# robin-karlsson0/pc-accumulation-lib

Hardware: AMD Instinct MI355X
Metric: Mpoints/s projected+accumulated and BEV frames/s @256x256; 1/2/4/8 GPU (higher is better)
Workload: dtype f64; 1 GPU; KITTI-360 single forward cam, 120k pts/frame, 200 m horizon (~201 live frames, 5169634 stored pts), one 256x256x21 BEV per integrated frame; points_per_frame=120000, bev_px=256, view_m=80

## Files before the change

### include/pca.h

```cpp
#ifndef PCA_H
#define PCA_H

#include <stdint.h>

#ifdef __cplusplus
extern "C" {
#endif

#define PCA_VERSION 2

typedef struct pca_ctx pca_ctx;

typedef struct {
    double *x, *y, *z;
    float *intensity;
    uint32_t *rgbs;
    int32_t *inst;
    uint8_t *dyn;
    int64_t capacity;
    uint32_t *frame_box;
} pca_store;

#define PCA_STATUS_STORE_OVERFLOW 1u
#define PCA_STATUS_UV_OUT_OF_IMAGE 2u
#define PCA_STATUS_NEGATIVE_INTENSITY 4u
#define PCA_STATUS_LOOKBACK_TIMEOUT 8u
#define PCA_STATUS_LANES_BISECT_CAP 16u

int pca_version(void);
int pca_ctx_create(int device, pca_ctx **out);
void pca_ctx_destroy(pca_ctx *ctx);
const char *pca_last_error(pca_ctx *ctx);
int pca_status(pca_ctx *ctx, void *stream, uint32_t *status_out);
int pca_status_peek(pca_ctx *ctx, uint32_t *status_out);
const uint32_t *pca_status_mirror(pca_ctx *ctx);

typedef struct {
    const float *pts;
    const uint8_t *rgb;
    const uint8_t *sem;
    const uint8_t *sem_gt;
    int32_t n;
    int32_t reserved;
} pca_kitti_frame;

int pca_kitti_project_sample_filter(pca_ctx *ctx, const pca_kitti_frame *frames, int n_frames, const double P[12],
                                    int H, int W, const uint64_t filter_mask[4], const pca_store *store,
                                    int64_t *frame_off , int first_slot, void *stream);

#define PCA_SAMPLE_NEAREST 0
#define PCA_SAMPLE_BILINEAR 1
int pca_kitti_project_sample_filter_ex(pca_ctx *ctx, const pca_kitti_frame *frames, int n_frames, const double P[12],
                                       int H, int W, const uint64_t filter_mask[4], const pca_store *store,
                                       int64_t *frame_off , int first_slot, int sample_mode, void *stream);

int pca_nusc_sample_filter_transform(pca_ctx *ctx, const double *pc, const int64_t *cam_idx, int32_t n,
                                     const uint8_t *imgs, const uint8_t *sems, int ncam, int H, int W,
                                     const double T[16], const uint64_t filter_mask[4], const pca_store *store,
                                     int64_t *frame_off , int slot, void *stream);
int pca_nusc_sample_filter_transform_ex(pca_ctx *ctx, const double *pc, const int64_t *cam_idx, int32_t n,
                                        const uint8_t *imgs, const uint8_t *sems, int ncam, int H, int W,
                                        const double T[16], const uint64_t filter_mask[4], const pca_store *store,
                                        int64_t *frame_off , int slot, int sample_mode, void *stream);

typedef struct {
    const double *pc;
    const int64_t *cam_idx;
    const uint8_t *imgs;
    const uint8_t *sems;
    int32_t n;
    int32_t reserved;
    const double *T;
} pca_nusc_frame;
int pca_nusc_sample_filter_transform_batch(pca_ctx *ctx, const pca_nusc_frame *frames, int n_frames, int ncam, int H, int W,
                                           const uint64_t filter_mask[4], const pca_store *store, int64_t *frame_off ,
                                           int first_slot, int sample_mode, void *stream);

int pca_sample_bilinear(pca_ctx *ctx, const double *map , int H, int W, const double *uv , int32_t n,
                        double *out , void *stream);

int pca_nusc_project_cams(pca_ctx *ctx, const double *pc_lidar, int32_t n, const double T_ego_from_lidar[16],
                          const double T_glob_from_ego[16], const double *T_cam_from_glob, const double *K,
                          const double *wh, int ncam, double *pc_in_ego, double *uv, int64_t *cam_idx,
                          void *stream);

#define PCA_NUSC_MAX_SWEEPS 32
#define PCA_NUSC_MAX_SWEEP_BOXES 4096
#define PCA_NUSC_MAX_SWEEP_TILES 16384
typedef struct {
    int32_t row0, n_rows;
    int32_t box0, n_boxes;
    float lag, sweep;
    double T[12];
} pca_nusc_sweep;
typedef struct {
    double inv[12];
    double size[3];
    int32_t cls;
    int32_t track_key;
} pca_nusc_sweep_box;
int64_t pca_nusc_merge_sweeps_workspace_bytes(int64_t n_points, int n_boxes);
int pca_nusc_merge_sweeps(pca_ctx *ctx, const float *raw , int64_t n_points, const pca_nusc_sweep *sweeps,
                          int n_sweeps, const pca_nusc_sweep_box *boxes, int n_boxes, float center_radius,
                          double inside_limit, void *workspace , int64_t workspace_bytes,
                          float *points_out , int32_t *tally_out , void *stream);

int pca_retransform(pca_ctx *ctx, const pca_store *store, const int64_t *frame_off , int slot_begin,
                    int slot_end, const double *Ts, int n_T, void *stream);

int pca_retransform_batch_tail(pca_ctx *ctx, const pca_store *store, const int64_t *frame_off , int first_slot,
                               int n_frames, const double *Ts, void *stream);

int pca_mark_dynamic(pca_ctx *ctx, const pca_store *store, const int64_t *frame_off , const int32_t *slots,
                     const int32_t *inst_idx, int n_pairs, void *stream);

int64_t pca_voxel_dedup_workspace_bytes(int64_t max_points, int n_slots);
int pca_voxel_dedup(pca_ctx *ctx, const pca_store *store, int64_t *frame_off , int slot_begin, int slot_end,
                    double voxel_size, int64_t max_points, void *workspace , int64_t workspace_bytes,
                    void *stream);

int64_t pca_icp_workspace_bytes(int32_t max_points);
int pca_icp_register(pca_ctx *ctx, const float *src_pts , int32_t n_src, const float *tgt_pts ,
                     int32_t n_tgt, double max_corr_dist, const double init[16], int max_iter, double rel_fitness,
                     double rel_rmse, void *workspace , int64_t workspace_bytes, double T_out[16],
                     double *fitness, double *rmse, int *iterations, void *stream);

typedef struct {
    double origin[3];
    double R[9];
    double dx, dy;
    double view;
    double height_filter;
    double int_scaler, int_sep_scaler, int_mid_threshold;
    double rgb_fill;
    int32_t px;
    int32_t road_class;
    uint64_t dynobj_mask[4];
    int32_t intensity_div255;
    int32_t pad;
} pca_bev_params;

int64_t pca_bev_workspace_bytes(int64_t max_points, int px);

int pca_bev_generate(pca_ctx *ctx, const pca_store *store, const double *intensity64,
                     const int64_t *frame_off , int slot_begin, int slot_split, int slot_end,
                     int64_t max_points, const pca_bev_params *prm, const double *pending_T, int pending_slot_end,
                     void *workspace , int64_t workspace_bytes, double *planes ,
                     uint16_t *planes_f16 , void *stream);

#define PCA_BEV_EXTRA_PLANES 3
int pca_bev_generate_ex(pca_ctx *ctx, const pca_store *store, const double *intensity64,
                        const int64_t *frame_off , int slot_begin, int slot_split, int slot_end,
                        int64_t max_points, const pca_bev_params *prm, const double *pending_T, int pending_slot_end,
                        void *workspace , int64_t workspace_bytes, double *planes ,
                        uint16_t *planes_f16 , double *extra_planes , void *stream);

#define PCA_BEV_MAX_CHAIN 4
int pca_bev_generate_chain(pca_ctx *ctx, const pca_store *store, const double *intensity64,
                           const int64_t *frame_off , int slot_begin, int slot_split, int slot_end,
                           int64_t max_points, const pca_bev_params *prm, const double *pending_Ts,
                           const int *pending_slot_ends, int n_pending, int write_back, void *workspace ,
                           int64_t workspace_bytes, double *planes , uint16_t *planes_f16 ,
                           double *extra_planes , void *stream);

typedef struct {
    int32_t slot_begin, slot_split, slot_end, reserved;
    pca_bev_params prm;
    double *planes;
    uint16_t *planes_f16;
} pca_bev_job;
int pca_bev_generate_many(pca_ctx *ctx, const pca_store *store, const double *intensity64 ,
                          const int64_t *frame_off , const pca_bev_job *jobs, int n_jobs, int64_t max_points,
                          void *workspace , int64_t workspace_bytes, void *stream);

#define PCA_BEV_MAX_CLASS_GROUPS 16
typedef struct { uint64_t mask[4]; } pca_class_group;
int64_t pca_bev_class_workspace_bytes(int64_t max_points, int px);
int pca_bev_class_planes(pca_ctx *ctx, const pca_store *store, const int64_t *frame_off ,
                         int slot_begin, int slot_split, int slot_end, int64_t max_points,
                         const pca_bev_params *prm,
                         const pca_class_group *groups, int n_groups,
                         const double *pending_Ts, const int *pending_slot_ends, int n_pending,
                         void *workspace , int64_t workspace_bytes,
                         double *prob      ,
                         uint16_t *prob_f16,
                         uint32_t *counts  ,
                         void *stream);

int64_t pca_bev_elev_workspace_bytes(int64_t max_points, int px);
int pca_bev_elev_partition(pca_ctx *ctx, const pca_store *store, const int64_t *frame_off ,
                           int slot_begin, int slot_end, int64_t max_points,
                           const pca_bev_params *prm, double elev_thresh, int include_dyn,
                           const double *pending_Ts, const int *pending_slot_ends, int n_pending,
                           void *workspace , int64_t workspace_bytes,
                           double *elev      ,
                           uint8_t *observed ,
                           uint8_t *flags    ,
                           int64_t *counts   ,
                           void *stream);

int pca_image_to_nchw_f32(pca_ctx *ctx, const uint8_t *rgb , int H, int W, const float mean[3], const float std[3],
                          float *out , void *stream);

int pca_bev_warp(pca_ctx *ctx, const uint16_t *planes_f16 , uint16_t *out_f16 , int n_planes, int px,
                 double a_1, double a_2, double b_1, double b_2, void *stream);

int pca_host_ego_to_grid(const double *full, int F, const double R[9], double dx, double dy, double view, int px,
                         double *rows, int32_t *start);

typedef struct {
    double origin[3];
    double R[9];
    double dx, dy, view;
    int32_t px, reserved;
} pca_lane_view;
int64_t pca_lanes_workspace_bytes(int64_t n_vertices, int n_samples, int64_t cap_rows);
int pca_lanes_transform(pca_ctx *ctx, double *xyz , int64_t P, const double T[16], void *stream);
int pca_lanes_to_grid(pca_ctx *ctx, const double *xyz , const int32_t *vertex_lane , const int32_t *start ,
                      int64_t P, int32_t L, const pca_lane_view *views , int S, int64_t cap_rows,
                      double *rows , int32_t *row_lane , int64_t *n_rows , void *ws,
                      void *stream);

typedef struct pca_host_track pca_host_track;
typedef struct {
    const void *pts;
    const void *rgb;
    const void *sem;
    const void *sem_gt;
    int32_t n;
    uint32_t host_mask;
} pca_kitti_obs;
int pca_kitti_integrate(pca_ctx *ctx, const pca_kitti_obs *obs, const double P[12], int H, int W,
                        const uint64_t filter_mask[4], const pca_store *store, int64_t *frame_off , int slot,
                        int sample_mode, pca_host_track *track, const double *T_new_prev, double horizon, int64_t *evicted,
                        double *path_length, void *stream);
void pca_host_camera_cone(const double P[12], int H, int W, double cone[15]);
int pca_host_view_hull(int F, const double *then , const float *box , const double *cone ,
                       const double now[12], const pca_bev_params *prm, int *first, int *last);
int pca_bev_bin_range(pca_ctx *ctx, int slot_first, int slot_last_plus1);
int pca_bev_view_hint(pca_ctx *ctx, int slot0, int F, const double *then, const float *box, const double *cone, const double now[12],
                      const pca_bev_params *prm);
void pca_f32_box_decode(const uint32_t *rows , int n, float *box );

int pca_debug_bev_level1(const pca_ctx *ctx, int out[4]);
int pca_debug_icp_layout(int32_t n_src, int32_t n_tgt, int64_t out[16]);

int pca_k1_defer(pca_ctx *ctx, int on);
int pca_k1_flush(pca_ctx *ctx);
int pca_kitti_generate_bev(pca_ctx *ctx, const pca_store *store, const int64_t *frame_off , int slot_begin,
                           int slot_split, int slot_end, int64_t max_points, const pca_bev_params *prm,
                           const double *pending_Ts, const int *pending_slot_ends, int n_pending, int write_back,
                           void *workspace , int64_t workspace_bytes, uint16_t *planes_f16 ,
                           void *host_planes , const pca_host_track *track, double *traj_rows,
                           int32_t *traj_start, int32_t *n_rows, void *stream);

typedef struct {
    const pca_kitti_obs *obs; const double *P; int32_t H, W; const uint64_t *filter_mask; const pca_store *store;
    int64_t *frame_off; int32_t slot, sample_mode; pca_host_track *track; const double *T_new_prev; double horizon;
    int64_t evicted; double path_length; void *stream;
} pca_kitti_integrate_args;
int pca_kitti_integrate_v(pca_ctx *ctx, pca_kitti_integrate_args *a);
typedef struct {
    const pca_store *store; const int64_t *frame_off; int32_t slot_begin, slot_split, slot_end, pad0; int64_t max_points;
    const pca_bev_params *prm; const double *pending_Ts; const int *pending_slot_ends; int32_t n_pending, write_back;
    void *workspace; int64_t workspace_bytes; uint16_t *planes_f16; void *host_planes; const pca_host_track *track;
    double *traj_rows; int32_t *traj_start; int32_t n_rows, pad1; void *stream;
    int32_t hint_slot0, hint_F; const double *hint_then; const float *hint_box; const double *hint_cone; const double *hint_now;
    int32_t hinted, pad2;
} pca_kitti_generate_bev_args;
int pca_kitti_generate_bev_v(pca_ctx *ctx, pca_kitti_generate_bev_args *a);

int pca_host_stage_h2d(int n, const void *const *src, void *const *pinned, void *const *dev, const int64_t *bytes,
                       void *stream);

int pca_host_d2h_async(pca_ctx *ctx, const void *dev, void *pinned, int64_t bytes, void *stream);
int pca_host_d2h_wait(pca_ctx *ctx, int ticket);

#define PCA_DEFLATE_CHUNK_MAX 32768
#define PCA_DEFLATE_MAX_CHUNKS (1 << 20)
#define PCA_DEFLATE_BOUND(n) ((9 * (int64_t)(n) + 7) / 8 + 16)
typedef struct { int64_t offset; int32_t length; int32_t reserved; } pca_deflate_chunk;
int64_t pca_deflate_workspace_bytes(int64_t n_chunks);
int pca_deflate_chunks(pca_ctx *ctx, const void *src , const pca_deflate_chunk *chunk_table , int64_t n_chunks,
                       void *out , uint32_t *out_sizes , uint32_t *out_crcs , void *workspace ,
                       void *stream);
uint32_t pca_host_crc32_combine(uint32_t crc_a, uint32_t crc_b, int64_t len_b);
int64_t pca_host_gzip_assemble(int32_t n_pieces, const void *const *piece, const int64_t *piece_bytes, const int64_t *raw_bytes,
                               const uint32_t *crc, void *out, int64_t out_cap);

typedef struct pca_host_track pca_host_track;
int pca_host_gemv4_probe(void *cblas_dgemv64, int mode, const double *T , const double *x , int64_t n,
                         double *y );
int pca_host_gemv4_mode(int mode);
int pca_host_incr_probe(void *cblas_dgemv64, const double *d, int64_t n, int64_t r0, int64_t r1, double *out);
int pca_host_incr_blocks(int on);
int pca_host_track_create(pca_host_track **out, void *cblas_dgemv64);
void pca_host_track_destroy(pca_host_track *t);
int64_t pca_host_track_len(const pca_host_track *t);
int64_t pca_host_track_n_segments(const pca_host_track *t);
const double *pca_host_track_poses(const pca_host_track *t);
const double *pca_host_track_segments(const pca_host_track *t);
int pca_host_track_set(pca_host_track *t, const double *poses , int64_t n, const double *segs, int64_t nd);
int pca_host_track_transform(pca_host_track *t, const double T[16]);
int pca_host_track_append(pca_host_track *t, const double pose[3]);
int pca_host_track_push_segment(pca_host_track *t, double *path_length);
int pca_host_track_incr(pca_host_track *t, double *out);
int64_t pca_host_track_evict_beyond(pca_host_track *t, double horizon, double path_length);
int64_t pca_host_track_step(pca_host_track *t, const double T_new_prev[16], double horizon, double *path_length);
int64_t pca_host_track_trigger(pca_host_track *t, double bev_horizon, int64_t previous_idx, double min_step);

enum {
    PCA_K_KITTI = 0, PCA_K_NUSC, PCA_K_PROJECT_CAMS, PCA_K_RETRANSFORM, PCA_K_MARK_DYNAMIC,
    PCA_K_BEV_BIN, PCA_K_BEV_SCAN, PCA_K_BEV_SCATTER, PCA_K_BEV_CELLS, PCA_K_BEV_CELLS_HEAVY, PCA_K_DEDUP, PCA_K_BEV_UNIT, PCA_K_ICP,
    PCA_K_BEV_CLASS_BIN, PCA_K_BEV_CLASS_CELLS, PCA_K_BEV_ELEV_BIN, PCA_K_BEV_ELEV_CELLS, PCA_K_COUNT
};
int pca_profile_enable(pca_ctx *ctx, int on);
int pca_profile_read(pca_ctx *ctx, int kernel_id, double *total_ms, int64_t *launches);

#ifdef __cplusplus
}
#endif
#endif
```

### pc-accumulation-lib_amd/csrc/pca_session.hip

```cpp
#include <vector>

#include "pca_common.h"

int pca_stage_copy(const void *const *src, void *const *dst, const int64_t *bytes, int n);

extern "C" {

int pca_kitti_integrate(pca_ctx *ctx, const pca_kitti_obs *obs, const double P[12], int H, int W,
                        const uint64_t filter_mask[4], const pca_store *store, int64_t *frame_off, int slot, int sample_mode,
                        pca_host_track *track, const double *T_new_prev, double horizon, int64_t *evicted,
                        double *path_length, void *stream)
{
    if (!ctx) return -1;
    if (!obs || obs->n < 0 || !P || !filter_mask || !store || !frame_off) { ctx->err = "kitti_integrate: bad arguments"; return -1; }
    if (track && (!T_new_prev || !evicted || !path_length)) { ctx->err = "kitti_integrate: the pose track needs T_new_prev and its outputs"; return -1; }
    hipStream_t s = (hipStream_t)stream;
    PCA_CHECK(ctx, hipSetDevice(ctx->device));
    if (pca_k1_flush_pending(ctx)) return -1;
    const void *in[4] = {obs->pts, obs->rgb, obs->sem, obs->sem_gt};
    const int64_t size[4] = {16ll * obs->n, 3ll * H * W, 1ll * H * W, 1ll * obs->n};
    const void *dev[4] = {in[0], in[1], in[2], in[3]};
    int64_t off[4] = {0, 0, 0, 0}, total = 0;
    for (int k = 0; k < 4; ++k) {
        if (!(in[k] && ((obs->host_mask >> k) & 1u))) continue;
        if (size[k] > 0) { off[k] = total; total += pca_align256(size[k]); }
        else dev[k] = nullptr;
    }
    pca_ctx::Stage *slot_st = nullptr;
    if (total > 0) {
        pca_ctx::Stage &st = ctx->stage[ctx->stage_next++ % PCA_STAGE_DEPTH];
        if (st.busy) { PCA_CHECK(ctx, hipEventSynchronize(st.done)); st.busy = false; }
        if (st.cap < total) {
            if (st.pin) PCA_CHECK(ctx, hipHostFree(st.pin));
            if (st.dev) PCA_CHECK(ctx, hipFree(st.dev));
            st.pin = st.dev = nullptr; st.cap = 0;
            const int64_t cap = total + total / 4;
            PCA_CHECK(ctx, hipHostMalloc(&st.pin, (size_t)cap));
            PCA_CHECK(ctx, hipMalloc(&st.dev, (size_t)cap));
            st.cap = cap;
        }
        if (!st.done) PCA_CHECK(ctx, hipEventCreateWithFlags(&st.done, hipEventDisableTiming));
        const void *src[4]; void *dst[4]; int64_t bytes[4]; int m = 0;
        for (int k = 0; k < 4; ++k)
            if (in[k] && ((obs->host_mask >> k) & 1u) && size[k] > 0) {
                src[m] = in[k]; dst[m] = (char *)st.pin + off[k]; bytes[m] = size[k]; ++m;
                dev[k] = (char *)st.dev + off[k];
            }
        pca_stage_copy(src, dst, bytes, m);
        const int64_t side_min = PCA_ENV_ONCE("PCA_H2D_SIDE_MIN", 256ll << 10);
        if (total >= side_min) {
            if (!ctx->h2d_stream[0]) PCA_CHECK(ctx, hipStreamCreateWithFlags(&ctx->h2d_stream[0], hipStreamNonBlocking));
            if (!ctx->h2d_done[0]) PCA_CHECK(ctx, hipEventCreateWithFlags(&ctx->h2d_done[0], hipEventDisableTiming));
            PCA_CHECK(ctx, hipMemcpyAsync(st.dev, st.pin, (size_t)total, hipMemcpyHostToDevice, ctx->h2d_stream[0]));
            PCA_CHECK(ctx, hipEventRecord(ctx->h2d_done[0], ctx->h2d_stream[0]));
            PCA_CHECK(ctx, hipStreamWaitEvent(s, ctx->h2d_done[0], 0));
        } else {
            PCA_CHECK(ctx, hipMemcpyAsync(st.dev, st.pin, (size_t)total, hipMemcpyHostToDevice, s));
        }
        slot_st = &st;
    }
    pca_kitti_frame fr;
    fr.pts = (const float *)dev[0]; fr.rgb = (const uint8_t *)dev[1]; fr.sem = (const uint8_t *)dev[2];
    fr.sem_gt = (const uint8_t *)dev[3]; fr.n = obs->n; fr.reserved = 0;
    const bool plain = obs->n > 0 && sample_mode == PCA_SAMPLE_NEAREST && (fr.sem_gt || ((int64_t)H * W * 3 >= 4 && fr.rgb && fr.sem)) &&
                       obs->n <= (1 << 20);
    if (ctx->k1_defer && plain) {
        pca_ctx::K1Pending &pd = ctx->k1_pend;
        pd.fr = fr;
        for (int i = 0; i < 12; ++i) pd.P[i] = P[i];
        pd.H = H; pd.W = W;
        for (int i = 0; i < 4; ++i) pd.filt[i] = filter_mask[i];
        pd.store = *store; pd.frame_off = frame_off; pd.slot = slot; pd.sample_mode = sample_mode; pd.stream = s;
        pd.stage_idx = slot_st ? (int)(slot_st - ctx->stage) : -1;
        pd.valid = true;
    } else {
        const int rc = pca_kitti_project_sample_filter_ex(ctx, &fr, 1, P, H, W, filter_mask, store, frame_off, slot, sample_mode, stream);
        if (slot_st) {
            const hipError_t e = hipEventRecord(slot_st->done, s);
            if (e == hipSuccess) slot_st->busy = true;
            else {
                (void)hipStreamSynchronize(s);
                if (rc == 0) { ctx->err = std::string("kitti_integrate: hipEventRecord(stage done): ") + hipGetErrorString(e); return -1; }
            }
        }
        if (rc != 0) return rc;
    }
    if (track) *evicted = pca_host_track_step(track, T_new_prev, horizon, path_length);
    return 0;
}

int pca_kitti_generate_bev(pca_ctx *ctx, const pca_store *store, const int64_t *frame_off, int slot_begin, int slot_split,
                           int slot_end, int64_t max_points, const pca_bev_params *prm, const double *pending_Ts,
                           const int *pending_slot_ends, int n_pending, int write_back, void *workspace,
                           int64_t workspace_bytes, uint16_t *planes_f16, void *host_planes, const pca_host_track *track,
                           double *traj_rows, int32_t *traj_start, int32_t *n_rows, void *stream)
{
    if (!ctx) return -1;
    if (!prm || !planes_f16 || !track || !traj_rows || !traj_start || !n_rows) { ctx->err = "kitti_generate_bev: bad arguments"; return -1; }
    const int64_t F = pca_host_track_len(track);
    if (F != slot_end - slot_begin) { ctx->err = "kitti_generate_bev: the pose track and the window disagree about the number of frames"; return -1; }
    static thread_local std::vector<double> rel;
    rel.resize((size_t)(3 * (F > 0 ? F : 1)));
    const double *Hp = pca_host_track_poses(track);
    for (int64_t f = 0; f < F; ++f)
        for (int k = 0; k < 3; ++k) rel[(size_t)(3 * f + k)] = Hp[4 * f + k] - prm->origin[k];
    *n_rows = pca_host_ego_to_grid(rel.data(), (int)F, prm->R, prm->dx, prm->dy, prm->view, prm->px, traj_rows, traj_start);
    if (pca_bev_generate_chain(ctx, store, nullptr, frame_off, slot_begin, slot_split, slot_end, max_points, prm, pending_Ts,
                               pending_slot_ends, n_pending, write_back, workspace, workspace_bytes, nullptr, planes_f16,
                               nullptr, stream) != 0)
        return -1;
    if (!host_planes) return 0;
    return pca_host_d2h_async(ctx, planes_f16, host_planes, 21ll * prm->px * prm->px * 2, stream);
}

int pca_kitti_integrate_v(pca_ctx *ctx, pca_kitti_integrate_args *a)
{
    if (!ctx) return -1;
    if (!a) { ctx->err = "kitti_integrate_v: no argument block"; return -1; }
    return pca_kitti_integrate(ctx, a->obs, a->P, a->H, a->W, a->filter_mask, a->store, a->frame_off, a->slot, a->sample_mode,
                               a->track, a->T_new_prev, a->horizon, &a->evicted, &a->path_length, a->stream);
}

int pca_kitti_generate_bev_v(pca_ctx *ctx, pca_kitti_generate_bev_args *a)
{
    if (!ctx) return -1;
    if (!a) { ctx->err = "kitti_generate_bev_v: no argument block"; return -1; }
    a->hinted = 0;
    if (a->hint_F > 0 && !(a->n_pending > 0 && a->write_back)) {
        const int rc = pca_bev_view_hint(ctx, a->hint_slot0, a->hint_F, a->hint_then, a->hint_box, a->hint_cone, a->hint_now, a->prm);
        if (rc < 0) { ctx->err = "kitti_generate_bev_v: bad view hint"; return -1; }
        a->hinted = rc;
    }
    return pca_kitti_generate_bev(ctx, a->store, a->frame_off, a->slot_begin, a->slot_split, a->slot_end, a->max_points, a->prm,
                                  a->pending_Ts, a->pending_slot_ends, a->n_pending, a->write_back, a->workspace,
                                  a->workspace_bytes, a->planes_f16, a->host_planes, a->track, a->traj_rows, a->traj_start,
                                  &a->n_rows, a->stream);
}

}
```

### pc-accumulation-lib_amd/kitti360_sem_pc_accum.py

```python
import os

import numpy as np

from sem_pc_accum import SemanticPointCloudAccumulator

_MODS = None


def _mods():
    global _MODS
    if _MODS is None:
        import ctypes

        import torch
        from bev_generator.sem_bev import LazyBev, SemBEVGenerator, _PendingCopy
        from pca_amd import host_logic
        from pca_amd._lib import PcaKittiObs
        _MODS = (ctypes, torch, LazyBev, _PendingCopy, SemBEVGenerator, host_logic, PcaKittiObs)
    return _MODS


class Kitti360SemanticPointCloudAccumulator(SemanticPointCloudAccumulator):

    def __init__(self, horizon_dist: float, calib_params: dict, icp_threshold: float, semseg_onnx_path: str,
                 semseg_filters: list, sem_idxs: dict, use_gt_sem: bool, bev_params: dict):
        super().__init__(horizon_dist, icp_threshold, semseg_onnx_path, semseg_filters, sem_idxs, use_gt_sem,
                         bev_params)
        self.H_velo_cam = calib_params['h_velo_cam']
        self.P_cam_frame = calib_params['p_cam_frame']
        self.P_velo_frame = calib_params['p_velo_frame']
        self._gpu_icp = None
        self._uploader = None
        self._cobs = None
        self._ga = None
        self._ga_traj = None
        self._fast = os.environ.get('PCA_FAST_CALLS', '1') != '0'
        self._defer_k1 = self._fast and os.environ.get('PCA_FUSE_K1', '1') != '0'
        self._prev_sweep = None
        self._sweep_dev = None
        self.pose_provider = self._default_pose_provider()

    def _default_pose_provider(self):
        import os
        path = os.environ.get('PCA_KITTI_T_FILE')
        if path:
            Ts = iter(np.load(path))
            return lambda pc: next(Ts)
        spec = os.environ.get('PCA_POSE_PROVIDER')
        if spec == 'gpu_icp':
            return self._gpu_icp_pose
        if spec == 'open3d':
            return self._icp_pose
        if spec:
            import importlib
            mod, _, fn = spec.partition(':')
            return getattr(importlib.import_module(mod), fn)
        return self._icp_pose

    def _gpu_icp_pose(self, pc):
        import torch
        from pca_amd.icp import GpuIcp
        if self._gpu_icp is None:
            self._gpu_icp = GpuIcp()
        if not isinstance(pc, torch.Tensor) and getattr(pc, 'dtype', None) == np.float32 and pc.ndim == 2 and pc.shape[1] == 4:
            new = self._upload([('icp_pts', pc)])[0]
            self._sweep_dev = (pc, new)
        else:
            new = GpuIcp.to_device(pc)
        if self._prev_sweep is None:
            self._prev_sweep = new
        reg = self._gpu_icp.register(self._prev_sweep, new, self.icp_threshold, self.icp_trans_init)
        self._prev_sweep = new
        return reg.transformation

    def _icp_pose(self, pc):
        try:
            import open3d as o3d
        except ImportError as e:
            raise ImportError('the KITTI-360 flow takes its poses from Open3D ICP, as the reference does, and open3d is '
                              'not importable; name another pose source: accumulator.pose_provider = callable, '
                              'PCA_KITTI_T_FILE=<poses.npy>, PCA_POSE_PROVIDER=<module>:<callable> or '
                              'PCA_POSE_PROVIDER=gpu_icp (device ICP, not bit-compatible with Open3D)') from e
        pcd_new = self.pc2pcd(pc)
        if self.pcd_prev is None:
            self.pcd_prev = pcd_new
        reg = o3d.pipelines.registration.registration_icp(
            self.pcd_prev, pcd_new, self.icp_threshold, self.icp_trans_init,
            o3d.pipelines.registration.TransformationEstimationPointToPlane())
        self.pcd_prev = pcd_new
        return reg.transformation

    def _frame_tensors(self, rgb, pc, sem_gt):
        import torch
        dev = self.store.device
        dtype_np = {torch.float32: np.float32, torch.uint8: np.uint8}
        want, host = {}, []

        def up(name, a, dtype):
            a = getattr(a, 'dev', a)
            if isinstance(a, torch.Tensor):
                if a.device != dev or a.dtype != dtype or not a.is_contiguous():
                    a = a.to(device=dev, dtype=dtype).contiguous()
                want[name] = a
            else:
                want[name] = len(host)
                host.append((name, np.ascontiguousarray(a, dtype=dtype_np[dtype])))

        up('pts', pc, torch.float32)
        semseg = None
        if sem_gt is None:
            img = rgb if isinstance(rgb, torch.Tensor) or hasattr(rgb, 'dev') else np.asarray(rgb)
            up('rgb', img, torch.uint8)
            if getattr(self.semseg_model, 'accepts_device', False):
                if not isinstance(want['rgb'], torch.Tensor):
                    want['rgb'] = self._upload(host[want['rgb']:want['rgb'] + 1])[0]
                    host.pop()
                semseg = self.semseg_model.pred(want['rgb'])[0, 0]
            else:
                semseg = self.semseg_model.pred(rgb)[0, 0]
            up('sem', semseg, torch.uint8)
        else:
            sg = sem_gt if isinstance(sem_gt, torch.Tensor) else np.asarray(sem_gt)[:, -1]
            up('sem_gt', sg, torch.uint8)
        if host:
            for (name, _), t in zip(host, self._upload(host)):
                want[name] = t
        frame = want
        H, W = tuple(frame['sem'].shape) if sem_gt is None else (1, 1)
        return frame, semseg, H, W

    def _upload(self, items):
        if self._uploader is None:
            from pca_amd.ingest import PinnedUploader
            self._uploader = PinnedUploader(self.store.device)
        return self._uploader.upload_many(items)

    def _obs_pointers(self, rgb, pc, sem_gt):
        _, torch, _, _, _, _, PcaKittiObs = _mods()
        dev = self.store.device
        obs = self._cobs
        if obs is None:
            obs = self._cobs = PcaKittiObs()
        keep, mask = [], 0

        def put(a, np_dtype, t_dtype, bit):
            nonlocal mask
            if not isinstance(a, torch.Tensor):
                own = getattr(a, '__dict__', {})
                d = own.get('dev') if isinstance(own.get('dev'), torch.Tensor) else own.get('_dev')
                if isinstance(d, torch.Tensor):
                    a = d
                elif '_host' in own and '_dev' in own:
                    a = a.host
            if isinstance(a, torch.Tensor):
                if a.device != dev or a.dtype != t_dtype or not a.is_contiguous():
                    a = a.to(device=dev, dtype=t_dtype).contiguous()
                keep.append(a)
                return a.data_ptr(), tuple(a.shape)
            a = np.ascontiguousarray(a, dtype=np_dtype)
            keep.append(a)
            mask |= bit
            return a.ctypes.data, a.shape

        obs.pts, shape = put(pc, np.float32, torch.float32, 1)
        if len(shape) != 2 or shape[1] != 4:
            raise ValueError('pc must be (N, 4): x, y, z, intensity')
        obs.n = int(shape[0])
        semseg = None
        if sem_gt is None:
            if getattr(self.semseg_model, 'accepts_device', False) and not isinstance(rgb, torch.Tensor) \
                    and getattr(rgb, '__dict__', {}).get('_dev') is None:
                return None
            obs.rgb, ishape = put(rgb, np.uint8, torch.uint8, 2)
            src = keep[-1] if getattr(self.semseg_model, 'accepts_device', False) else rgb
            semseg = self.semseg_model.pred(src)[0, 0]
            obs.sem, sshape = put(semseg, np.uint8, torch.uint8, 4)
            if len(ishape) != 3 or ishape[2] != 3 or tuple(ishape[:2]) != tuple(sshape):
                raise ValueError(f'image {tuple(ishape)} and class map {tuple(sshape)} do not fit together')
            obs.sem_gt = None
            H, W = int(sshape[0]), int(sshape[1])
        else:
            sg = sem_gt if isinstance(sem_gt, torch.Tensor) else np.asarray(sem_gt)[:, -1]
            obs.sem_gt, gshape = put(sg, np.uint8, torch.uint8, 8)
            if tuple(gshape) != (obs.n, ):
                raise ValueError('sem_gt must hold one label per point')
            obs.rgb = obs.sem = None
            H, W = 1, 1
        obs.host_mask = mask
        return obs, semseg, H, W, keep

    def integrate(self, observations: list):
        rgb, pc, sem_gt = observations[0]
        if not self.use_gt_sem:
            sem_gt = None
        T_new_prev = np.asarray(self.pose_provider(pc), dtype=np.float64)
        self.T_prev_origin = np.matmul(self.T_prev_origin, T_new_prev)
        if self._sweep_dev is not None:
            host, dev = self._sweep_dev
            self._sweep_dev = None
            if host is pc:
                pc = dev
        fast = self._obs_pointers(rgb, pc, sem_gt) if self._fast else None
        general = self._frame_tensors(rgb, pc, sem_gt) if fast is None else None
        if len(self._track) > 0:
            self.update_sem_pcs(T_new_prev)
        if fast is not None:
            obs, semseg, H, W, keep = fast
            if self._defer_k1 != getattr(self.store.ctx, 'k1_defer', False):
                self.store.set_defer_k1(self._defer_k1)
            idx, path_length = self.store.append_kitti_obs(obs, self.P_velo_frame, H, W, self.semseg_filters, self.sample_mode,
                                                           self._track, T_new_prev, self.horizon_dist, keep=keep)
            del keep
            if idx is None:
                idx, path_length = self._track.step(T_new_prev, self.horizon_dist)
        else:
            frame, semseg, H, W = general
            self.store.append_kitti([frame], self.P_velo_frame, H, W, self.semseg_filters, sample_mode=self.sample_mode)
            idx, path_length = self._track.step(T_new_prev, self.horizon_dist)
        self.rgbs.append(rgb)
        self.semsegs.append(semseg)
        if idx:
            self.store.evict(idx)
            self.rgbs = self.rgbs[idx:]
            self.semsegs = self.semsegs[idx:]
        if path_length is not None:
            print(f'    #pc {self.store.n_frames} |', f'path length {path_length:.2f}')
        self._after_integrate()
        return idx

    def integrate_many(self, batch: list, max_frames_per_launch: int = 64):
        if self.voxel_dedup:
            return [self.integrate(obs) for obs in batch]
        out = []
        for b0 in range(0, len(batch), max_frames_per_launch):
            out += self._integrate_batch(batch[b0:b0 + max_frames_per_launch])
        return out

    def _integrate_batch(self, batch):
        from pca_amd.ingest import check_ring_lifetime
        check_ring_lifetime([item for observations in batch for item in observations[0]], len(batch))
        frames, Ts, shape = [], [], None
        for observations in batch:
            rgb, pc, sem_gt = observations[0]
            if not self.use_gt_sem:
                sem_gt = None
            T_new_prev = np.asarray(self.pose_provider(pc), dtype=np.float64)
            self.T_prev_origin = np.matmul(self.T_prev_origin, T_new_prev)
            if self._sweep_dev is not None:
                host, dev = self._sweep_dev
                self._sweep_dev = None
                if host is pc:
                    pc = dev
            frame, semseg, H, W = self._frame_tensors(rgb, pc, sem_gt)
            if shape not in (None, (H, W)):
                raise ValueError('integrate_many: all images of a batch must have one size')
            shape = (H, W)
            frames.append(frame)
            Ts.append(T_new_prev)
            self.rgbs.append(rgb)
            self.semsegs.append(semseg)
        self.store.flush_pending()
        self.store.append_kitti(frames, self.P_velo_frame, shape[0], shape[1], self.semseg_filters,
                                sample_mode=self.sample_mode)
        self.store.retransform_batch(np.stack(Ts), len(frames))
        removed, total = [], 0
        for T_new_prev in Ts:
            idx, path_length = self._track.step(T_new_prev, self.horizon_dist)
            if path_length is not None:
                print(f'    #pc {len(self._track)} |', f'path length {path_length:.2f}')
            removed.append(idx)
            total += idx
            self._integrated += 1
        self.store.poll_status()
        if total:
            self.store.evict(total)
            self.rgbs = self.rgbs[total:]
            self.semsegs = self.semsegs[total:]
        return removed

    def obs2sem_vec_space(self, rgb, pc, sem_gt=None) -> tuple:
        from pca_amd.device_store import DeviceStore
        T_new_prev = np.asarray(self.pose_provider(pc), dtype=np.float64)
        self.T_prev_origin = np.matmul(self.T_prev_origin, T_new_prev)
        main, self._store = self._store, DeviceStore(capacity=max(len(pc), 1), max_frames=2)
        try:
            frame, semseg, H, W = self._frame_tensors(rgb, pc, sem_gt)
            self._store.append_kitti([frame], self.P_velo_frame, H, W, self.semseg_filters)
            rows = self._store.rows(0)
        finally:
            self._store = main
        return rows, [0., 0., 0.], semseg, T_new_prev

    def generate_bev(self, present_idx: int = None, bev_num: int = 1, gen_future: bool = False):
        if bev_num == 1 and gen_future and self._fast_bev_ok(present_idx):
            return [self._generate_bev_fast(present_idx)]
        pcs, trajs = self._window_inputs(present_idx, gen_future)
        return self._run_bev(pcs, trajs, bev_num)

    def generate_bev_device(self, present_idx: int, out=None):
        if self._fast_bev_ok(present_idx):
            return self._generate_bev_fast(present_idx, out=out, to_host=False)
        pcs, trajs = self._window_inputs(present_idx, True)
        return self.sem_bev_generator.generate(pcs, trajs, device_only=True, out=out)

    def _fast_bev_ok(self, present_idx):
        gen = self.sem_bev_generator
        if not self._fast or type(gen) is not _mods()[4] or gen.do_aug or gen.do_warp or self._store is None \
                or getattr(self._track, '_h', None) is None or os.environ.get('PCA_SYNC_BEV') or getattr(gen, 'sem_planes', None):
            return False
        if not isinstance(present_idx, (int, np.integer)):
            return False
        n = self._store.n_frames
        split = int(present_idx) if present_idx >= 0 else n + int(present_idx)
        return 0 < split < n and n == len(self._track)

    def _generate_bev_fast(self, present_idx, out=None, to_host=True):
        C, torch, LazyBev, _PendingCopy, _, hl, _ = _mods()
        st, gen, track = self.store, self.sem_bev_generator, self._track
        ctx = st.ctx
        st.poll_status()
        n = st.n_frames
        present_idx = int(present_idx)
        split = present_idx if present_idx >= 0 else n + present_idx
        lo = max(split - 2, 0)
        near = track.poses_window(lo, split + 1)
        origin = near[split - lo]
        rot_mat = hl.rotation_matrix_3d(hl.heading_rot_ang(near[:split - lo] - origin))
        px = gen.pixel_size
        prm = gen._raster_params(origin, rot_mat, 0., 0., 1. * gen.view_size, st.intensity_div255)
        max_points = st.bev_workspace(px)
        n_pend, pend_T, pend_ends, write_back = st.bev_pending(0, n)
        if out is None:
            out = torch.empty((21, px, px), dtype=torch.float16, device=st.device)
        else:
            assert out.dtype == torch.float16 and out.is_contiguous() and tuple(out.shape) == (21, px, px)
        host = torch.empty((1, 21, px, px), dtype=torch.float16, pin_memory=True) if to_host else None
        tb = self._ga_traj
        if tb is None or tb[0].shape[0] < 2 * n or tb[1].shape[0] < n + 1:
            tb = self._ga_traj = (np.empty((4 * n + 64, 3)), np.zeros(2 * n + 64, dtype=np.int32))
            self._ga_traj_addr = (tb[0].ctypes.data, tb[1].ctypes.data)
        start = tb[1]
        cst = st.c_store()
        a = self._ga
        if a is None:
            from pca_amd._lib import PcaKittiGenerateBevArgs
            a = self._ga = PcaKittiGenerateBevArgs()
            self._ga_const = None
        pend_T, pend_ends = st._pend_T, st._pend_ends
        const = (id(cst), id(st.frame_off), id(prm), id(pend_T), id(pend_ends), id(st._ws), track._h)
        if const != self._ga_const:
            a.store, a.frame_off, a.prm = C.addressof(cst), st.frame_off.data_ptr(), C.addressof(prm)
            a.pending_Ts, a.pending_slot_ends = C.addressof(pend_T), C.addressof(pend_ends)
            a.workspace, a.workspace_bytes = st._ws.data_ptr(), st._ws.numel()
            a.track = getattr(track._h, 'value', track._h)
            self._ga_const = const
            self._ga_keep = (cst, st.frame_off, prm, pend_T, pend_ends, st._ws)
        a.slot_begin, a.slot_split, a.slot_end, a.max_points = st.head, st.head + split, st.head + n, max_points
        a.n_pending, a.write_back = n_pend, write_back
        a.planes_f16, a.host_planes = out.data_ptr(), (None if host is None else host.data_ptr())
        a.traj_rows, a.traj_start = self._ga_traj_addr
        a.stream = ctx.stream_int() or None
        a.hint_F = st.view_hint_into(a, 0, n)
        ticket = ctx.lib.pca_kitti_generate_bev_v(ctx.h, C.addressof(a))
        if ticket < 0:
            ctx.check(ticket)
        st.hints_taken += a.hinted
        st.bev_done(write_back)
        rows = tb[0][:a.n_rows].copy()
        empty = np.zeros((0, 3))
        ego_p = rows[:start[split - 1]].copy() if split >= 2 else empty
        ego_f = rows[start[split]:].copy() if n - split >= 2 else empty
        if not to_host:
            return {'planes_f16': out, 'trajs_present': [ego_p], 'trajs_future': [ego_f], 'trajs_full': [rows]}
        return LazyBev(host, 0, _PendingCopy(ctx, ticket, (out, host)), ([ego_p], [ego_f], [rows]))
```

### pc-accumulation-lib_amd/pca_amd/_lib.py

```python
import ctypes as C
import os
import threading

import numpy as np

_HERE = os.path.dirname(os.path.abspath(__file__))
LIB_PATH = os.path.join(_HERE, 'libpca_hip.so')

STATUS_STORE_OVERFLOW = 1
STATUS_UV_OUT_OF_IMAGE = 2
STATUS_NEGATIVE_INTENSITY = 4
STATUS_LOOKBACK_TIMEOUT = 8
STATUS_LANES_BISECT_CAP = 16
SAMPLE_MODES = {'nearest': 0, 'bilinear': 1}

EXPORTS = ('pca_version', 'pca_ctx_create', 'pca_ctx_destroy', 'pca_last_error', 'pca_status', 'pca_status_peek', 'pca_status_mirror',
           'pca_kitti_project_sample_filter', 'pca_kitti_project_sample_filter_ex',
           'pca_nusc_sample_filter_transform', 'pca_nusc_sample_filter_transform_ex', 'pca_nusc_sample_filter_transform_batch', 'pca_sample_bilinear', 'pca_nusc_project_cams',
           'pca_nusc_merge_sweeps_workspace_bytes', 'pca_nusc_merge_sweeps', 'pca_retransform', 'pca_retransform_batch_tail',
           'pca_mark_dynamic',
           'pca_bev_workspace_bytes', 'pca_bev_generate', 'pca_bev_generate_ex', 'pca_bev_generate_chain', 'pca_bev_generate_many', 'pca_bev_class_workspace_bytes', 'pca_bev_class_planes', 'pca_bev_elev_workspace_bytes', 'pca_bev_elev_partition', 'pca_bev_warp', 'pca_lanes_workspace_bytes', 'pca_lanes_transform', 'pca_lanes_to_grid', 'pca_image_to_nchw_f32', 'pca_voxel_dedup_workspace_bytes', 'pca_voxel_dedup', 'pca_icp_workspace_bytes', 'pca_icp_register', 'pca_host_ego_to_grid',
           'pca_host_gemv4_probe', 'pca_host_gemv4_mode', 'pca_host_incr_probe', 'pca_host_incr_blocks', 'pca_host_track_create', 'pca_host_track_destroy', 'pca_host_track_len', 'pca_host_track_n_segments',
           'pca_host_track_poses', 'pca_host_track_segments', 'pca_host_track_set', 'pca_host_track_transform',
           'pca_host_track_append', 'pca_host_track_push_segment', 'pca_host_track_incr', 'pca_host_track_evict_beyond',
           'pca_host_track_step', 'pca_host_track_trigger', 'pca_host_stage_h2d', 'pca_host_d2h_async', 'pca_host_d2h_wait',
           'pca_deflate_workspace_bytes', 'pca_deflate_chunks', 'pca_host_crc32_combine', 'pca_host_gzip_assemble',
           'pca_kitti_integrate', 'pca_kitti_generate_bev', 'pca_k1_defer', 'pca_k1_flush', 'pca_host_camera_cone', 'pca_host_view_hull', 'pca_bev_bin_range', 'pca_bev_view_hint', 'pca_kitti_integrate_v', 'pca_kitti_generate_bev_v', 'pca_f32_box_decode', 'pca_debug_bev_level1', 'pca_debug_icp_layout',
           'pca_profile_enable', 'pca_profile_read')

KERNEL_IDS = ('kitti_project_sample_filter', 'nusc_sample_filter_transform', 'nusc_project_cams', 'retransform',
              'mark_dynamic', 'bev_bin', 'bev_scan', 'bev_scatter', 'bev_cells', 'bev_cells_heavy', 'voxel_dedup', 'bev_unit', 'icp', 'bev_class_bin', 'bev_class_cells', 'bev_elev_bin', 'bev_elev_cells')
BEV_EXTRA_PLANES = ('elevation_max', 'elevation_mean', 'intensity_mean')


class PcaStore(C.Structure):
    _fields_ = [('x', C.c_void_p), ('y', C.c_void_p), ('z', C.c_void_p), ('intensity', C.c_void_p),
                ('rgbs', C.c_void_p), ('inst', C.c_void_p), ('dyn', C.c_void_p), ('capacity', C.c_int64),
                ('frame_box', C.c_void_p)]


class PcaKittiIntegrateArgs(C.Structure):
    _fields_ = [('obs', C.c_void_p), ('P', C.c_void_p), ('H', C.c_int32), ('W', C.c_int32), ('filter_mask', C.c_void_p),
                ('store', C.c_void_p), ('frame_off', C.c_void_p), ('slot', C.c_int32), ('sample_mode', C.c_int32),
                ('track', C.c_void_p), ('T_new_prev', C.c_void_p), ('horizon', C.c_double), ('evicted', C.c_int64),
                ('path_length', C.c_double), ('stream', C.c_void_p)]


class PcaKittiGenerateBevArgs(C.Structure):
    _fields_ = [('store', C.c_void_p), ('frame_off', C.c_void_p), ('slot_begin', C.c_int32), ('slot_split', C.c_int32),
                ('slot_end', C.c_int32), ('pad0', C.c_int32), ('max_points', C.c_int64), ('prm', C.c_void_p),
                ('pending_Ts', C.c_void_p), ('pending_slot_ends', C.c_void_p), ('n_pending', C.c_int32), ('write_back', C.c_int32),
                ('workspace', C.c_void_p), ('workspace_bytes', C.c_int64), ('planes_f16', C.c_void_p), ('host_planes', C.c_void_p),
                ('track', C.c_void_p), ('traj_rows', C.c_void_p), ('traj_start', C.c_void_p), ('n_rows', C.c_int32),
                ('pad1', C.c_int32), ('stream', C.c_void_p), ('hint_slot0', C.c_int32), ('hint_F', C.c_int32),
                ('hint_then', C.c_void_p), ('hint_box', C.c_void_p), ('hint_cone', C.c_void_p), ('hint_now', C.c_void_p),
                ('hinted', C.c_int32), ('pad2', C.c_int32)]


class PcaKittiObs(C.Structure):
    _fields_ = [('pts', C.c_void_p), ('rgb', C.c_void_p), ('sem', C.c_void_p), ('sem_gt', C.c_void_p),
                ('n', C.c_int32), ('host_mask', C.c_uint32)]


class PcaKittiFrame(C.Structure):
    _fields_ = [('pts', C.c_void_p), ('rgb', C.c_void_p), ('sem', C.c_void_p), ('sem_gt', C.c_void_p),
                ('n', C.c_int32), ('reserved', C.c_int32)]


class PcaNuscFrame(C.Structure):
    _fields_ = [('pc', C.c_void_p), ('cam_idx', C.c_void_p), ('imgs', C.c_void_p), ('sems', C.c_void_p),
                ('n', C.c_int32), ('reserved', C.c_int32), ('T', C.POINTER(C.c_double))]


class PcaBevParams(C.Structure):
    _fields_ = [('origin', C.c_double * 3), ('R', C.c_double * 9), ('dx', C.c_double), ('dy', C.c_double),
                ('view', C.c_double), ('height_filter', C.c_double), ('int_scaler', C.c_double),
                ('int_sep_scaler', C.c_double), ('int_mid_threshold', C.c_double), ('rgb_fill', C.c_double),
                ('px', C.c_int32), ('road_class', C.c_int32), ('dynobj_mask', C.c_uint64 * 4),
                ('intensity_div255', C.c_int32), ('pad', C.c_int32)]


class PcaClassGroup(C.Structure):
    _fields_ = [('mask', C.c_uint64 * 4)]


BEV_MAX_CLASS_GROUPS = 16


class PcaBevJob(C.Structure):
    _fields_ = [('slot_begin', C.c_int32), ('slot_split', C.c_int32), ('slot_end', C.c_int32), ('reserved', C.c_int32),
                ('prm', PcaBevParams), ('planes', C.c_void_p), ('planes_f16', C.c_void_p)]


def class_mask(classes):
    m = [0, 0, 0, 0]
    for c in classes or []:
        c = int(c)
        if 0 <= c < 256:
            m[c >> 6] |= 1 << (c & 63)
    return (C.c_uint64 * 4)(*m)


def f64_array(a, n):
    a = np.ascontiguousarray(a, dtype=np.float64).ravel()
    assert a.size == n, (a.size, n)
    return (C.c_double * n)(*a.tolist())


_lib = None


def load():
    global _lib
    if _lib is not None:
        return _lib
    if not os.path.exists(LIB_PATH):
        raise RuntimeError(f'{LIB_PATH} not found: build it with `python -c "import __graft_entry__ as g; '
                           f'g.build()"` or `make -C pc-accumulation-lib_amd/csrc` (no CPU fallback exists)')
    import torch
    lib = C.CDLL(LIB_PATH)
    vp, i32, i64 = C.c_void_p, C.c_int, C.c_int64
    lib.pca_version.restype = C.c_int
    lib.pca_ctx_create.argtypes = [i32, C.POINTER(vp)]
    lib.pca_ctx_destroy.argtypes = [vp]
    lib.pca_ctx_destroy.restype = None
    lib.pca_last_error.argtypes = [vp]
    lib.pca_last_error.restype = C.c_char_p
    lib.pca_status.argtypes = [vp, vp, C.POINTER(C.c_uint32)]
    lib.pca_status_peek.argtypes = [vp, C.POINTER(C.c_uint32)]
    lib.pca_status_mirror.argtypes = [vp]
    lib.pca_status_mirror.restype = vp
    lib.pca_kitti_project_sample_filter.argtypes = [
        vp, C.POINTER(PcaKittiFrame), i32, C.POINTER(C.c_double), i32, i32, C.POINTER(C.c_uint64),
        C.POINTER(PcaStore), vp, i32, vp
    ]
    lib.pca_kitti_project_sample_filter_ex.argtypes = [
        vp, C.POINTER(PcaKittiFrame), i32, C.POINTER(C.c_double), i32, i32, C.POINTER(C.c_uint64),
        C.POINTER(PcaStore), vp, i32, i32, vp
    ]
    lib.pca_nusc_sample_filter_transform_ex.argtypes = [
        vp, vp, vp, C.c_int32, vp, vp, i32, i32, i32, C.POINTER(C.c_double), C.POINTER(C.c_uint64),
        C.POINTER(PcaStore), vp, i32, i32, vp
    ]
    lib.pca_nusc_sample_filter_transform_batch.argtypes = [
        vp, C.POINTER(PcaNuscFrame), i32, i32, i32, i32, C.POINTER(C.c_uint64), C.POINTER(PcaStore), vp, i32, i32, vp
    ]
    lib.pca_sample_bilinear.argtypes = [vp, vp, i32, i32, vp, C.c_int32, vp, vp]
    lib.pca_nusc_sample_filter_transform.argtypes = [
        vp, vp, vp, C.c_int32, vp, vp, i32, i32, i32, C.POINTER(C.c_double), C.POINTER(C.c_uint64),
        C.POINTER(PcaStore), vp, i32, vp
    ]
    lib.pca_nusc_project_cams.argtypes = [
        vp, vp, C.c_int32, C.POINTER(C.c_double), C.POINTER(C.c_double), C.POINTER(C.c_double),
        C.POINTER(C.c_double), C.POINTER(C.c_double), i32, vp, vp, vp, vp
    ]
    lib.pca_nusc_merge_sweeps_workspace_bytes.argtypes = [i64, i32]
    lib.pca_nusc_merge_sweeps_workspace_bytes.restype = i64
    lib.pca_nusc_merge_sweeps.argtypes = [vp, vp, i64, vp, i32, vp, i32, C.c_float, C.c_double, vp, i64, vp, vp, vp]
    lib.pca_retransform.argtypes = [vp, C.POINTER(PcaStore), vp, i32, i32, C.POINTER(C.c_double), i32, vp]
    lib.pca_retransform_batch_tail.argtypes = [vp, C.POINTER(PcaStore), vp, i32, i32, C.POINTER(C.c_double), vp]
    lib.pca_mark_dynamic.argtypes = [vp, C.POINTER(PcaStore), vp, C.POINTER(C.c_int32), C.POINTER(C.c_int32), i32, vp]
    lib.pca_bev_workspace_bytes.argtypes = [i64, i32]
    lib.pca_bev_workspace_bytes.restype = i64
    lib.pca_bev_generate.argtypes = [
        vp, C.POINTER(PcaStore), vp, vp, i32, i32, i32, i64, C.POINTER(PcaBevParams), C.POINTER(C.c_double), i32,
        vp, i64, vp, vp, vp
    ]
    lib.pca_bev_generate_ex.argtypes = [
        vp, C.POINTER(PcaStore), vp, vp, i32, i32, i32, i64, C.POINTER(PcaBevParams), C.POINTER(C.c_double), i32,
        vp, i64, vp, vp, vp, vp
    ]
    lib.pca_image_to_nchw_f32.argtypes = [vp, vp, i32, i32, C.POINTER(C.c_float), C.POINTER(C.c_float), vp, vp]
    a = list(lib.pca_bev_generate_ex.argtypes)
    lib.pca_bev_generate_chain.argtypes = a[:9] + [vp, vp, i32, i32] + a[11:]
    lib.pca_bev_generate_many.argtypes = [vp, C.POINTER(PcaStore), vp, vp, C.POINTER(PcaBevJob), i32, i64, vp, i64, vp]
    lib.pca_bev_class_workspace_bytes.argtypes = [i64, i32]
    lib.pca_bev_class_workspace_bytes.restype = i64
    lib.pca_bev_class_planes.argtypes = [vp, C.POINTER(PcaStore), vp, i32, i32, i32, i64, C.POINTER(PcaBevParams),
                                         C.POINTER(PcaClassGroup), i32, vp, vp, i32, vp, i64, vp, vp, vp, vp]
    lib.pca_bev_elev_workspace_bytes.argtypes = [i64, i32]
    lib.pca_bev_elev_workspace_bytes.restype = i64
    lib.pca_bev_elev_partition.argtypes = [vp, C.POINTER(PcaStore), vp, i32, i32, i64, C.POINTER(PcaBevParams), C.c_double, i32,
                                           vp, vp, i32, vp, i64, vp, vp, vp, vp, vp]
    lib.pca_bev_warp.argtypes = [vp, vp, vp, i32, i32, C.c_double, C.c_double, C.c_double, C.c_double, vp]
    lib.pca_voxel_dedup_workspace_bytes.restype = C.c_int64
    lib.pca_voxel_dedup_workspace_bytes.argtypes = [i64, i32]
    lib.pca_voxel_dedup.argtypes = [vp, C.POINTER(PcaStore), vp, i32, i32, C.c_double, i64, vp, i64, vp]
    lib.pca_icp_workspace_bytes.restype = C.c_int64
    lib.pca_icp_workspace_bytes.argtypes = [i32]
    lib.pca_icp_register.argtypes = [vp, vp, i32, vp, i32, C.c_double, C.POINTER(C.c_double), i32, C.c_double,
                                     C.c_double, vp, i64, C.POINTER(C.c_double), C.POINTER(C.c_double),
                                     C.POINTER(C.c_double), C.POINTER(C.c_int), vp]
    lib.pca_host_ego_to_grid.argtypes = [vp, i32, vp, C.c_double, C.c_double, C.c_double, i32, vp, vp]
    lib.pca_lanes_workspace_bytes.argtypes = [i64, i32, i64]
    lib.pca_lanes_workspace_bytes.restype = i64
    lib.pca_lanes_transform.argtypes = [vp, vp, i64, vp, vp]
    lib.pca_lanes_to_grid.argtypes = [vp, vp, vp, vp, i64, C.c_int32, vp, i32, i64, vp, vp, vp, vp, vp]
    dp = C.POINTER(C.c_double)
    lib.pca_host_gemv4_probe.argtypes = [vp, i32, vp, vp, i64, vp]
    lib.pca_host_gemv4_mode.argtypes = [i32]
    lib.pca_host_incr_probe.argtypes = [vp, vp, i64, i64, i64, vp]
    lib.pca_host_incr_blocks.argtypes = [i32]
    lib.pca_host_track_create.argtypes = [C.POINTER(vp), vp]
    lib.pca_host_track_destroy.argtypes = [vp]
    lib.pca_host_track_destroy.restype = None
    for name in ('pca_host_track_len', 'pca_host_track_n_segments'):
        getattr(lib, name).argtypes = [vp]
        getattr(lib, name).restype = i64
    for name in ('pca_host_track_poses', 'pca_host_track_segments'):
        getattr(lib, name).argtypes = [vp]
        getattr(lib, name).restype = vp
    lib.pca_host_track_set.argtypes = [vp, vp, i64, vp, i64]
    lib.pca_host_track_transform.argtypes = [vp, vp]
    lib.pca_host_track_append.argtypes = [vp, vp]
    lib.pca_host_track_push_segment.argtypes = [vp, dp]
    lib.pca_host_track_incr.argtypes = [vp, vp]
    lib.pca_host_track_evict_beyond.argtypes = [vp, C.c_double, C.c_double]
    lib.pca_host_track_evict_beyond.restype = i64
    lib.pca_host_track_step.argtypes = [vp, vp, C.c_double, dp]
    lib.pca_host_track_step.restype = i64
    lib.pca_host_track_trigger.argtypes = [vp, C.c_double, i64, C.c_double]
    lib.pca_host_track_trigger.restype = i64
    lib.pca_host_stage_h2d.argtypes = [i32, vp, vp, vp, vp, vp]
    lib.pca_host_d2h_async.argtypes = [vp, vp, vp, i64, vp]
    lib.pca_host_d2h_wait.argtypes = [vp, i32]
    lib.pca_deflate_workspace_bytes.argtypes = [i64]
    lib.pca_deflate_workspace_bytes.restype = i64
    lib.pca_deflate_chunks.argtypes = [vp, vp, vp, i64, vp, vp, vp, vp, vp]
    lib.pca_host_crc32_combine.argtypes = [C.c_uint32, C.c_uint32, i64]
    lib.pca_host_crc32_combine.restype = C.c_uint32
    lib.pca_host_gzip_assemble.argtypes = [i32, vp, vp, vp, vp, vp, i64]
    lib.pca_host_gzip_assemble.restype = i64
    lib.pca_kitti_integrate.argtypes = [vp, C.POINTER(PcaKittiObs), C.POINTER(C.c_double), i32, i32, C.POINTER(C.c_uint64),
                                        C.POINTER(PcaStore), vp, i32, i32, vp, vp, C.c_double, C.POINTER(C.c_int64),
                                        C.POINTER(C.c_double), vp]
    lib.pca_kitti_generate_bev.argtypes = [vp, C.POINTER(PcaStore), vp, i32, i32, i32, i64, C.POINTER(PcaBevParams), vp, vp,
                                           i32, i32, vp, i64, vp, vp, vp, vp, vp, C.POINTER(C.c_int32), vp]
    lib.pca_host_camera_cone.argtypes = [vp, i32, i32, vp]
    lib.pca_host_camera_cone.restype = None
    lib.pca_host_view_hull.argtypes = [i32, vp, vp, vp, vp, vp, C.POINTER(C.c_int), C.POINTER(C.c_int)]
    lib.pca_bev_bin_range.argtypes = [vp, i32, i32]
    lib.pca_bev_view_hint.argtypes = [vp, i32, i32, vp, vp, vp, vp, vp]
    lib.pca_f32_box_decode.argtypes = [vp, i32, vp]
    lib.pca_f32_box_decode.restype = None
    lib.pca_debug_bev_level1.argtypes = [vp, vp]
    lib.pca_debug_icp_layout.argtypes = [i32, i32, C.POINTER(C.c_int64)]
    lib.pca_kitti_integrate_v.argtypes = [vp, vp]
    lib.pca_kitti_generate_bev_v.argtypes = [vp, vp]
    lib.pca_k1_defer.argtypes = [vp, i32]
    lib.pca_k1_flush.argtypes = [vp]
    lib.pca_profile_enable.argtypes = [vp, i32]
    lib.pca_profile_read.argtypes = [vp, i32, C.POINTER(C.c_double), C.POINTER(C.c_int64)]
    _lib = lib
    return lib


class Context:

    _by_device = {}
    _raw_stream = None
    _tls = threading.local()

    def __init__(self, device_index):
        import torch
        if not torch.cuda.is_available():
            raise RuntimeError('pca_amd needs an AMD GPU (torch.cuda.is_available() is False); '
                               'there is no CPU fallback')
        self.lib = load()
        self.device_index = int(device_index)
        h = C.c_void_p()
        if self.lib.pca_ctx_create(self.device_index, C.byref(h)) != 0:
            raise RuntimeError('pca_ctx_create failed')
        self.h = h
        self._mirror = (C.c_uint32 * 8).from_address(self.lib.pca_status_mirror(h))
        self._mirror_q = (C.c_uint64 * 4).from_address(C.addressof(self._mirror))

    @classmethod
    def get(cls, device=None):
        import torch
        if not torch.cuda.is_available():
            raise RuntimeError('pca_amd needs an AMD GPU (torch.cuda.is_available() is False); '
                               'there is no CPU fallback')
        idx = torch.cuda.current_device() if device is None else torch.device(device).index or 0
        lane = getattr(cls._tls, 'lane', None)
        if lane is not None and lane.device_index == idx:
            return lane
        if idx not in cls._by_device:
            cls._by_device[idx] = Context(idx)
        return cls._by_device[idx]

    def destroy(self):
        if self.h is not None:
            self.lib.pca_ctx_destroy(self.h)
            self.h = None

    def stream(self):
        return C.c_void_p(self.stream_int())

    def stream_int(self):
        raw = self._raw_stream
        if raw is None:
            import torch
            raw = getattr(torch._C, '_cuda_getCurrentRawStream', None)
            if raw is None:
                return torch.cuda.current_stream(self.device_index).cuda_stream
            self._raw_stream = raw
        return raw(self.device_index)

    def check(self, rc):
        if rc != 0:
            raise RuntimeError('pca: ' + self.lib.pca_last_error(self.h).decode())

    def profile(self, on):
        self.check(self.lib.pca_profile_enable(self.h, int(on)))

    def profile_read(self):
        out = {}
        for k, name in enumerate(KERNEL_IDS):
            ms, n = C.c_double(0), C.c_int64(0)
            self.check(self.lib.pca_profile_read(self.h, k, C.byref(ms), C.byref(n)))
            out[name] = (ms.value, n.value)
        return out

    def peek_status(self):
        q = self._mirror_q
        if not (q[0] | q[1] | q[2] | q[3]):
            return 0
        m = self._mirror
        return sum(1 << b for b in range(8) if m[b])

    def check_status(self):
        st = self.status()
        if not st:
            return
        said = [(STATUS_UV_OUT_OF_IMAGE, AssertionError, 'pts_uv must be all inside image'),
                (STATUS_STORE_OVERFLOW, RuntimeError, 'pca: device point store overflow (points were dropped)'),
                (STATUS_LOOKBACK_TIMEOUT, RuntimeError,
                 'pca: a compaction workgroup timed out waiting for its predecessor (output invalid)'),
                (STATUS_NEGATIVE_INTENSITY, ValueError, 'pca: negative lidar intensity on the f32 path (pass intensity64 to bev())'),
                (STATUS_LANES_BISECT_CAP, RuntimeError, 'pca: a lane\'s border crossing was not found within the iteration cap (row invalid)')]
        hit = [(exc, msg) for bit, exc, msg in said if st & bit]
        rest = st & ~(STATUS_UV_OUT_OF_IMAGE | STATUS_STORE_OVERFLOW | STATUS_LOOKBACK_TIMEOUT | STATUS_NEGATIVE_INTENSITY | STATUS_LANES_BISECT_CAP)
        if rest:
            hit.append((RuntimeError, 'pca: unknown device status bits 0x%x' % rest))
        raise hit[0][0]('; '.join(msg for _, msg in hit))

    def poll_status(self):
        if self.peek_status():
            self.check_status()

    def status(self):
        st = C.c_uint32(0)
        self.check(self.lib.pca_status(self.h, self.stream(), C.byref(st)))
        return st.value


class Lane:

    def __init__(self, device=None, priority=0):
        import torch
        idx = torch.cuda.current_device() if device is None else torch.device(device).index or 0
        self.ctx = Context(idx)
        self.stream = torch.cuda.Stream(device=idx, priority=priority)
        self._guard = None
        self._outer = None

    def __enter__(self):
        import torch
        self._outer = getattr(Context._tls, 'lane', None)
        Context._tls.lane = self.ctx
        self._guard = torch.cuda.stream(self.stream)
        self._guard.__enter__()
        return self

    def __exit__(self, *exc):
        self._guard.__exit__(*exc)
        Context._tls.lane = self._outer
        self._guard = None
        return False

    def synchronize(self):
        self.stream.synchronize()

    def close(self):
        self.stream.synchronize()
        self.ctx.destroy()
```

### pc-accumulation-lib_amd/pca_amd/device_store.py

```python
import ctypes as C
import os

import numpy as np
import torch

from . import _lib
from ._lib import PcaBevParams, PcaKittiFrame, PcaStore

CULL = os.environ.get('PCA_BEV_CULL', '1') != '0'


class DeviceStore:
    CHAIN_MAX = 4
    CHAIN_K = int(os.environ.get('PCA_BEV_CHAIN', '4'))

    def __init__(self, capacity=1 << 24, max_frames=4096, device=None, intensity_div255=False):
        self.ctx = _lib.Context.get(device)
        self.device = torch.device('cuda', self.ctx.device_index)
        self.intensity_div255 = bool(intensity_div255)
        self.max_frames = int(max_frames)
        self._alloc(int(capacity))
        self.frame_off = torch.zeros(self.max_frames + 1, dtype=torch.int64, device=self.device)
        self._moved = np.eye(4)
        self.cull = CULL
        self.hints_taken = 0
        self._alloc_frame_tables(self.max_frames)
        self.head = 0
        self.tail = 0
        self.ub_tail = 0
        self.lb_head = 0
        self._ub = []
        self._ub_sum = 0
        self._pending = []
        self._k1_cache = None
        self._k1_src = None
        self._ia = None
        self._ws = None
        self._ws_many = None
        self._ws_points, self._ws_px = 0, 0
        self._ws_cls = None
        self._ws_cls_points, self._ws_cls_px = 0, 0
        self._ws_elev = None
        self._ws_elev_points, self._ws_elev_px = 0, 0
        self._dedup_ws = None
        self._obs_out = None
        self._k1_noted = None
        self._pend_T = (C.c_double * (16 * self.CHAIN_MAX))()
        self._pend_T_np = np.frombuffer(self._pend_T, dtype=np.float64)
        self._pend_ends = (C.c_int * self.CHAIN_MAX)()

    def _alloc(self, cap):
        d = self.device
        self.capacity = cap
        self._cstore = None
        self.x = torch.empty(cap, dtype=torch.float64, device=d)
        self.y = torch.empty(cap, dtype=torch.float64, device=d)
        self.z = torch.empty(cap, dtype=torch.float64, device=d)
        self.intensity = torch.empty(cap, dtype=torch.float32, device=d)
        self.rgbs = torch.empty(cap, dtype=torch.int32, device=d)
        self.inst = torch.empty(cap, dtype=torch.int32, device=d)
        self.dyn = torch.empty(cap, dtype=torch.uint8, device=d)

    def _arrays(self):
        return (self.x, self.y, self.z, self.intensity, self.rgbs, self.inst, self.dyn)

    BOX_EVERY = 16

    def _alloc_frame_tables(self, max_frames, keep=None):
        n1 = max_frames + 1
        box = torch.zeros((n1, 6), dtype=torch.int32, device=self.device)
        then = np.full((n1, 12), np.nan)
        seen = np.tile(np.array([1, -1] * 3, dtype=np.float32), (n1, 1))
        cone = np.zeros(n1, dtype=bool)
        if keep is not None:
            a, n = keep
            box[:n] = self.frame_box[a:a + n]
            then[:n], seen[:n], cone[:n] = self._then[a:a + n], self._box[a:a + n], self._has_cone[a:a + n]
        self.frame_box, self._then, self._box, self._has_cone = box, then, seen, cone
        self._then_addr, self._box_addr = then.ctypes.data, seen.ctypes.data
        self._box_pin = None
        self._box_copy = None
        self._since_box = 0
        self._cone = None
        self._n_nocone = 0 if keep is None else int(np.count_nonzero(~cone[:keep[1]] & np.isfinite(then[:keep[1], 0])))
        self._cstore = None

    def _note_moved(self, Ts):
        for T in Ts:
            M = T.reshape(4, 4) @ self._moved
            M[3] = (0., 0., 0., 1.)
            self._moved = M

    def _note_frame(self, slot, cone_key):
        self._then[slot] = self._moved[:3].reshape(12)
        if cone_key is not None:
            if self._cone is None or self._cone[0] != cone_key:
                if self._cone is not None:
                    self._has_cone[self.head:self.tail] = False
                    self._n_nocone = self.tail - self.head
                out = np.empty(15)
                Pm = np.frombuffer(cone_key[0], dtype=np.float64)
                self.ctx.lib.pca_host_camera_cone(Pm.ctypes.data, int(cone_key[1]), int(cone_key[2]), out.ctypes.data)
                self._cone = (cone_key, out, out.ctypes.data)
            self._has_cone[slot] = True
        else:
            self._n_nocone += 1
        self._since_box += 1
        self._poll_boxes()
        if self._since_box >= self.BOX_EVERY and self._box_copy is None:
            n = self.tail - self.head
            if n > 0:
                if self._box_pin is None or self._box_pin.shape[0] < self.frame_box.shape[0]:
                    self._box_pin = torch.empty(tuple(self.frame_box.shape), dtype=torch.int32, pin_memory=True)
                self._box_pin[:n].copy_(self.frame_box[self.head:self.tail], non_blocking=True)
                ev = torch.cuda.Event()
                ev.record()
                self._box_copy = (ev, self.head, n)
                self._since_box = 0

    def _poll_boxes(self):
        if self._box_copy is None or not self._box_copy[0].query():
            return
        _, first, n = self._box_copy
        self._box_copy = None
        rows = self._box_pin[:n].numpy()
        dec = np.empty((n, 6), dtype=np.float32)
        self.ctx.lib.pca_f32_box_decode(rows.ctypes.data, n, dec.ctypes.data)
        known = dec[:, 0] <= dec[:, 1]
        tgt = self._box[first:first + n]
        tgt[known] = dec[known]

    def view_hint_into(self, args, first_frame, last_frame):
        n = last_frame - first_frame
        if not self.cull or n < 4:
            return 0
        a = self.head + first_frame
        args.hint_slot0 = a
        args.hint_then, args.hint_box = self._then_addr + 96 * a, self._box_addr + 24 * a
        args.hint_cone = self._cone[2] if (self._cone is not None and self._n_nocone == 0) else None
        args.hint_now = self._moved.ctypes.data
        return n

    def view_hint(self, prm, first_frame, last_frame, write_back):
        n = last_frame - first_frame
        if not self.cull or write_back or n < 4:
            return 0
        a = self.head + first_frame
        cone = self._cone[2] if (self._cone is not None and self._n_nocone == 0) else None
        return self._count_hint(self.ctx.lib.pca_bev_view_hint(self.ctx.h, a, n, self._then_addr + 96 * a, self._box_addr + 24 * a, cone,
                                              self._moved.ctypes.data, C.addressof(prm)))

    def _count_hint(self, r):
        self.hints_taken += 1 if r > 0 else 0
        return r

    def c_store(self):
        if self._cstore is None:
            self._cstore = PcaStore(self.x.data_ptr(), self.y.data_ptr(), self.z.data_ptr(), self.intensity.data_ptr(),
                                    self.rgbs.data_ptr(), self.inst.data_ptr(), self.dyn.data_ptr(), self.capacity,
                                    self.frame_box.data_ptr())
        return self._cstore

    @property
    def n_frames(self):
        return self.tail - self.head

    def set_defer_k1(self, on):
        self.ctx.check(self.ctx.lib.pca_k1_defer(self.ctx.h, 1 if on else 0))
        self.ctx.k1_defer = bool(on)
        if not on:
            self._k1_noted = None

    def flush_k1(self):
        if self._k1_noted is not None:
            self.ctx.check(self.ctx.lib.pca_k1_flush(self.ctx.h))
            self._k1_noted = None

    def __del__(self):
        try:
            if self._k1_noted is not None:
                self.flush_k1()
        except Exception:
            pass

    def offsets(self):
        self.flush_k1()
        off = self.frame_off[self.head:self.tail + 1].cpu().numpy()
        self.lb_head = int(off[0])
        self.ub_tail = int(off[-1])
        self._ub = [int(v) for v in np.diff(off)]
        self._ub_sum = sum(self._ub)
        return off

    def sizes(self):
        return np.diff(self.offsets())

    def poll_status(self):
        self.ctx.poll_status()

    def check_status(self):
        self.ctx.check_status()

    def reserve(self, n_new, n_slots=1):
        if self.tail + n_slots <= self.max_frames and self.ub_tail + n_new <= self.capacity:
            return
        self.flush_pending()
        off = self.offsets()
        a, b = int(off[0]), int(off[-1])
        live, nf = b - a, self.n_frames
        new_cap = self.capacity
        while live + n_new > new_cap:
            new_cap *= 2
        new_maxf = self.max_frames
        while nf + n_slots > new_maxf:
            new_maxf *= 2
        old = self._arrays()
        if new_cap != self.capacity:
            self._alloc(new_cap)
            for dst, src in zip(self._arrays(), old):
                dst[:live] = src[a:b]
        elif a > 0:
            for t in old:
                t[:live] = t[a:b].clone()
        self.max_frames = new_maxf
        new_off = torch.zeros(new_maxf + 1, dtype=torch.int64, device=self.device)
        new_off[:nf + 1] = torch.from_numpy(off - a).to(self.device)
        self.frame_off = new_off
        cone = self._cone
        self._alloc_frame_tables(new_maxf, keep=(self.head, nf))
        self._cone = cone
        self.head, self.tail = 0, nf
        self.lb_head, self.ub_tail = 0, live

    def evict(self, k):
        k = int(k)
        if self._n_nocone and k:
            sl = slice(self.head, self.head + k)
            self._n_nocone -= int(np.count_nonzero(~self._has_cone[sl] & np.isfinite(self._then[sl, 0])))
        self.head += k
        self._ub_sum -= sum(self._ub[:int(k)])
        del self._ub[:int(k)]

    def max_window_points(self):
        return max(self._ub_sum, 1)

    def clear(self):
        self.flush_k1()
        self.head = self.tail = 0
        self.ub_tail = self.lb_head = 0
        self._ub = []
        self._ub_sum = 0
        self._pending = []
        self.frame_off.zero_()
        self._alloc_frame_tables(self.max_frames)
        self._moved = np.eye(4)

    @staticmethod
    def kitti_descs(frames):
        descs = (PcaKittiFrame * len(frames))()
        for k, f in enumerate(frames):
            n = int(f['pts'].shape[0])
            assert f['pts'].dtype == torch.float32 and f['pts'].is_contiguous()
            descs[k].pts = f['pts'].data_ptr() if n else None
            descs[k].rgb = f['rgb'].data_ptr() if f.get('rgb') is not None else None
            descs[k].sem = f['sem'].data_ptr() if f.get('sem') is not None else None
            descs[k].sem_gt = f['sem_gt'].data_ptr() if f.get('sem_gt') is not None else None
            descs[k].n = n
        return descs

    def append_kitti(self, frames, P, H, W, filters, descs=None, sample_mode='nearest'):
        lib, ctx = self.ctx.lib, self.ctx
        n_in = sum(int(f['pts'].shape[0]) for f in frames)
        self.reserve(n_in, len(frames))
        if descs is None:
            descs = self.kitti_descs(frames)
        st = self.c_store()
        key = (np.asarray(P, dtype=np.float64).tobytes(), tuple(int(c) for c in (filters or ())))
        if self._k1_cache is None or self._k1_cache[0] != key:
            self._k1_cache = (key, _lib.f64_array(P, 12), _lib.class_mask(filters))
        Pc, fmask = self._k1_cache[1], self._k1_cache[2]
        ctx.check(lib.pca_kitti_project_sample_filter_ex(ctx.h, descs, len(frames), Pc, int(H), int(W),
                                                         fmask, C.byref(st), self.frame_off.data_ptr(), self.tail,
                                                         _lib.SAMPLE_MODES[sample_mode], ctx.stream()))
        self.tail += len(frames)
        self.ub_tail += n_in
        self._ub += [int(f['pts'].shape[0]) for f in frames]
        self._ub_sum += n_in

    def append_kitti_obs(self, obs, P, H, W, filters, sample_mode='nearest', track=None, T_new_prev=None, horizon=0., keep=None):
        lib, ctx = self.ctx.lib, self.ctx
        n = int(obs.n)
        self.reserve(n, 1)
        src = self._k1_src
        if src is not None and src[0] is P and src[1] is filters and P.tobytes() == src[2] and tuple(filters or ()) == src[3]:
            key = self._k1_cache[0]
        else:
            key = (np.asarray(P, dtype=np.float64).tobytes(), tuple(int(c) for c in (filters or ())))
            ok = isinstance(P, np.ndarray) and P.dtype == np.float64 and all(type(c) is int for c in (filters or ()))
            self._k1_src = (P, filters, key[0], key[1]) if ok else None
        if self._k1_cache is None or self._k1_cache[0] != key:
            self._k1_cache = (key, _lib.f64_array(P, 12), _lib.class_mask(filters))
        Pc, fmask = self._k1_cache[1], self._k1_cache[2]
        st = self.c_store()
        th = getattr(track, '_h', None)
        a = self._ia
        if a is None:
            a = self._ia = _lib.PcaKittiIntegrateArgs()
            self._ia_T = np.zeros(16)
            self._ia_T_addr = self._ia_T.ctypes.data
            self._ia_const = None
        const = (id(obs), id(Pc), int(H), int(W), id(st), id(self.frame_off), sample_mode, th, float(horizon))
        if const != self._ia_const:
            a.obs, a.P, a.H, a.W, a.filter_mask = C.addressof(obs), C.addressof(Pc), int(H), int(W), C.addressof(fmask)
            a.store, a.frame_off, a.sample_mode = C.addressof(st), self.frame_off.data_ptr(), _lib.SAMPLE_MODES[sample_mode]
            a.track, a.horizon = getattr(th, 'value', th), float(horizon)
            self._ia_const = const
            self._ia_keep = (obs, Pc, fmask, st, self.frame_off)
        a.slot = self.tail
        if th is not None:
            self._ia_T[:] = np.asarray(T_new_prev, dtype=np.float64).reshape(16)
            a.T_new_prev = self._ia_T_addr
        else:
            a.T_new_prev = None
        a.stream = ctx.stream_int() or None
        ctx.check(lib.pca_kitti_integrate_v(ctx.h, C.addressof(a)))
        self._k1_noted = (keep, ) if getattr(ctx, 'k1_defer', False) else None
        self._note_frame(self.tail, (key[0], int(H), int(W)) if obs.sem_gt is None else None)
        self.tail += 1
        self.ub_tail += n
        self._ub.append(n)
        self._ub_sum += n
        if th is None:
            return None, None
        v = a.path_length
        return int(a.evicted), (None if v != v else np.float64(v))

    def append_nusc(self, pc, cam_idx, imgs, sems, T, filters, sample_mode='nearest'):
        lib, ctx = self.ctx.lib, self.ctx
        n = int(pc.shape[0])
        self.reserve(n)
        ncam, H, W = sems.shape
        st = self.c_store()
        ctx.check(lib.pca_nusc_sample_filter_transform_ex(ctx.h, pc.data_ptr(), cam_idx.data_ptr(), n, imgs.data_ptr(),
                                                          sems.data_ptr(), int(ncam), int(H), int(W),
                                                          _lib.f64_array(T, 16), _lib.class_mask(filters),
                                                          C.byref(st), self.frame_off.data_ptr(), self.tail,
                                                          _lib.SAMPLE_MODES[sample_mode], ctx.stream()))
        self.tail += 1
        self.ub_tail += n
        self._ub.append(n)
        self._ub_sum += n

    def append_nusc_many(self, frames, filters, sample_mode='nearest'):
        lib, ctx = self.ctx.lib, self.ctx
        if not frames:
            return
        ncam, H, W = (int(v) for v in frames[0]['sems'].shape)
        max_tiles = 16384
        b0 = 0
        while b0 < len(frames):
            tiles, b1 = 0, b0
            while b1 < len(frames):
                t = max((int(frames[b1]['pc'].shape[0]) + 511) // 512, 1)
                if b1 > b0 and tiles + t > max_tiles:
                    break
                tiles += t
                b1 += 1
            part = frames[b0:b1]
            n_in = sum(int(f['pc'].shape[0]) for f in part)
            self.reserve(n_in, len(part))
            descs = (_lib.PcaNuscFrame * len(part))()
            keep = []
            for k, f in enumerate(part):
                assert f['pc'].dtype == torch.float64 and f['pc'].is_contiguous() and f['cam_idx'].dtype == torch.int64
                assert tuple(f['sems'].shape) == (ncam, H, W) and f['imgs'].is_contiguous() and f['sems'].is_contiguous()
                n = int(f['pc'].shape[0])
                Tc = _lib.f64_array(f['T'], 16)
                keep.append(Tc)
                descs[k].pc = f['pc'].data_ptr() if n else None
                descs[k].cam_idx = f['cam_idx'].data_ptr() if n else None
                descs[k].imgs, descs[k].sems = f['imgs'].data_ptr(), f['sems'].data_ptr()
                descs[k].n = n
                descs[k].T = C.cast(Tc, C.POINTER(C.c_double))
            st = self.c_store()
            ctx.check(lib.pca_nusc_sample_filter_transform_batch(ctx.h, descs, len(part), ncam, H, W, _lib.class_mask(filters),
                                                                 C.byref(st), self.frame_off.data_ptr(), self.tail,
                                                                 _lib.SAMPLE_MODES[sample_mode], ctx.stream()))
            self.tail += len(part)
            self.ub_tail += n_in
            self._ub += [int(f['pc'].shape[0]) for f in part]
            self._ub_sum += n_in
            b0 = b1

    def retransform(self, Ts, defer=False):
        if self.n_frames == 0:
            return
        Ts = np.ascontiguousarray(Ts, dtype=np.float64).reshape(-1, 16)
        self._note_moved(Ts)
        if defer and Ts.shape[0] == 1:
            if len(self._pending) >= self.CHAIN_MAX:
                self.flush_pending()
            self._pending.append((Ts[0].copy(), self.tail))
            return
        self.flush_pending()
        self._launch_retransform(Ts, self.head, self.tail)

    def _launch_retransform(self, Ts, begin_slot, end_slot):
        st = self.c_store()
        ctx = self.ctx
        ctx.check(ctx.lib.pca_retransform(ctx.h, C.byref(st), self.frame_off.data_ptr(), begin_slot, end_slot,
                                          _lib.f64_array(Ts, Ts.size), Ts.shape[0], ctx.stream()))

    def retransform_batch(self, Ts, n_new):
        Ts = np.ascontiguousarray(Ts, dtype=np.float64).reshape(-1, 16)
        assert Ts.shape[0] == n_new
        self.flush_pending()
        self._note_moved(Ts)
        first_new = self.tail - n_new
        if first_new > self.head:
            st, ctx = self.c_store(), self.ctx
            ctx.check(ctx.lib.pca_retransform(ctx.h, C.byref(st), self.frame_off.data_ptr(), self.head, first_new,
                                              _lib.f64_array(Ts, Ts.size), Ts.shape[0], ctx.stream()))
        st, ctx = self.c_store(), self.ctx
        ctx.check(ctx.lib.pca_retransform_batch_tail(ctx.h, C.byref(st), self.frame_off.data_ptr(), first_new, n_new,
                                                     _lib.f64_array(Ts, Ts.size), ctx.stream()))

    def flush_pending(self):
        pend, self._pending = self._pending, []
        begin = self.head
        for k, (_, end_slot) in enumerate(pend):
            if end_slot > begin:
                self._launch_retransform(np.stack([T for T, _ in pend[k:]]), begin, end_slot)
                begin = end_slot

    def mark_dynamic(self, pairs):
        pairs = list(pairs)
        if not pairs:
            return
        slots = (C.c_int32 * len(pairs))(*[self.head + int(f) for f, _ in pairs])
        insts = (C.c_int32 * len(pairs))(*[int(i) for _, i in pairs])
        st = self.c_store()
        ctx = self.ctx
        ctx.check(ctx.lib.pca_mark_dynamic(ctx.h, C.byref(st), self.frame_off.data_ptr(), slots, insts, len(pairs),
                                           ctx.stream()))

    def voxel_dedup(self, voxel_size):
        if self.n_frames == 0:
            return
        self.flush_pending()
        ctx, lib = self.ctx, self.ctx.lib
        max_points = self.max_window_points()
        need = lib.pca_voxel_dedup_workspace_bytes(max_points, self.n_frames)
        if self._dedup_ws is None or self._dedup_ws.numel() < need:
            self._dedup_ws = torch.empty(int(need) + 256, dtype=torch.uint8, device=self.device)
        st = self.c_store()
        ctx.check(lib.pca_voxel_dedup(ctx.h, C.byref(st), self.frame_off.data_ptr(), self.head, self.tail,
                                      float(voxel_size), max_points, self._dedup_ws.data_ptr(),
                                      self._dedup_ws.numel(), ctx.stream()))

    def bev(self, split_frame, prm, want_f64=False, intensity64=None, first_frame=0, last_frame=None, out16=None,
            extra=None):
        ctx, lib = self.ctx, self.ctx.lib
        last_frame = self.n_frames if last_frame is None else last_frame
        px = int(prm.px)
        max_points = self.bev_workspace(px)
        if out16 is not None:
            assert out16.dtype == torch.float16 and out16.is_contiguous() and tuple(out16.shape) == (21, px, px)
        p16 = out16 if out16 is not None else torch.empty((21, px, px), dtype=torch.float16, device=self.device)
        p64 = torch.empty((21, px, px), dtype=torch.float64, device=self.device) if want_f64 else None
        st = self.c_store()
        n_pend, pend_T, pend_ends, write_back = self.bev_pending(first_frame, last_frame)
        if extra is not None:
            assert extra.dtype == torch.float64 and extra.is_contiguous() \
                and tuple(extra.shape) == (3, len(_lib.BEV_EXTRA_PLANES), px, px)
        self.view_hint(prm, first_frame, last_frame, n_pend > 0 and write_back)
        ctx.check(lib.pca_bev_generate_chain(ctx.h, C.byref(st), None if intensity64 is None else intensity64.data_ptr(),
                                             self.frame_off.data_ptr(), self.head + first_frame, self.head + split_frame,
                                             self.head + last_frame, max_points, C.byref(prm), pend_T, pend_ends, n_pend,
                                             write_back, self._ws.data_ptr(), self._ws.numel(),
                                             None if p64 is None else p64.data_ptr(), p16.data_ptr(),
                                             None if extra is None else extra.data_ptr(), ctx.stream()))
        self.bev_done(write_back)
        return p16, p64

    def bev_workspace(self, px):
        max_points = self.max_window_points()
        if self._ws is None or max_points > self._ws_points or px != self._ws_px:
            self._ws_points, self._ws_px = int(max_points * 1.25) + 1, px
            need = self.ctx.lib.pca_bev_workspace_bytes(self._ws_points, px)
            if self._ws is None or self._ws.numel() < need:
                self._ws = torch.empty(int(need) + 256, dtype=torch.uint8, device=self.device)
        return max_points

    def bev_pending(self, first_frame, last_frame):
        if not self._pending:
            return 0, None, None, 1
        if first_frame != 0 or self._pending[-1][1] > self.head + last_frame:
            self.flush_pending()
            return 0, None, None, 1
        n_pend = 0
        for T, e in self._pending:
            if e > self.head:
                self._pend_T_np[16 * n_pend:16 * n_pend + 16] = T
                self._pend_ends[n_pend] = int(e)
                n_pend += 1
        if n_pend == 0:
            return 0, None, None, 0
        return n_pend, self._pend_T, self._pend_ends, (1 if n_pend >= self.CHAIN_K else 0)

    def bev_done(self, write_back):
        if self._pending and write_back:
            self._pending = []
        self._k1_noted = None

    def bev_class_planes(self, split_frame, prm, groups, first_frame=0, last_frame=None, want_counts=False):
        ctx, lib = self.ctx, self.ctx.lib
        self.flush_k1()
        last_frame = self.n_frames if last_frame is None else last_frame
        px, ng = int(prm.px), len(groups)
        cg = (_lib.PcaClassGroup * max(ng, 1))()
        for k, g in enumerate(groups):
            cg[k].mask[:] = list(_lib.class_mask(g))
        n_pend, pend_T, pend_ends, _ = self.bev_pending(first_frame, last_frame)
        max_points = self.max_window_points()
        if self._ws_cls is None or max_points > self._ws_cls_points or px != self._ws_cls_px:
            self._ws_cls_points, self._ws_cls_px = int(max_points * 1.25) + 1, px
            need = lib.pca_bev_class_workspace_bytes(self._ws_cls_points, px)
            if self._ws_cls is None or self._ws_cls.numel() < need:
                self._ws_cls = torch.empty(int(need) + 256, dtype=torch.uint8, device=self.device)
        shape = (3, max(ng, 1), max(px, 1), max(px, 1))
        p16 = torch.empty(shape, dtype=torch.float16, device=self.device)
        p64 = torch.empty(shape, dtype=torch.float64, device=self.device)
        cnt = torch.empty((3, shape[1] + 1) + shape[2:], dtype=torch.int32, device=self.device) if want_counts else None
        st = self.c_store()
        ctx.check(lib.pca_bev_class_planes(ctx.h, C.byref(st), self.frame_off.data_ptr(), self.head + first_frame,
                                           self.head + split_frame, self.head + last_frame, max_points, C.byref(prm), cg, ng,
                                           pend_T, pend_ends, n_pend, self._ws_cls.data_ptr(), self._ws_cls.numel(),
                                           p64.data_ptr(), p16.data_ptr(), None if cnt is None else cnt.data_ptr(),
                                           ctx.stream()))
        return p16, p64, cnt

    def bev_elev_partition(self, prm, elev_thresh, first_frame=0, last_frame=None, include_dyn=False, mark_dyn=False,
                           max_points=None):
        ctx, lib = self.ctx, self.ctx.lib
        last_frame = self.n_frames if last_frame is None else last_frame
        px = int(prm.px)
        if mark_dyn:
            self.flush_pending()
        n_pend, pend_T, pend_ends, _ = self.bev_pending(first_frame, last_frame)
        bound = self.max_window_points()
        max_points = bound if max_points is None else max(int(max_points), 1)
        if self._ws_elev is None or max_points > self._ws_elev_points or px != self._ws_elev_px:
            self._ws_elev_points, self._ws_elev_px = int(max_points * 1.25) + 1, px
        need = lib.pca_bev_elev_workspace_bytes(self._ws_elev_points, px)
        if self._ws_elev is None or self._ws_elev.numel() < need:
            self._ws_elev = torch.empty(int(need) + 256, dtype=torch.uint8, device=self.device)
        side = max(px, 1)
        elev = torch.empty((side, side), dtype=torch.float64, device=self.device)
        obs = torch.empty((side, side), dtype=torch.uint8, device=self.device)
        flags = torch.empty(max_points, dtype=torch.uint8, device=self.device)
        counts = torch.empty(3, dtype=torch.int64, device=self.device)
        st = self.c_store()
        ctx.check(lib.pca_bev_elev_partition(ctx.h, C.byref(st), self.frame_off.data_ptr(), self.head + first_frame,
                                             self.head + last_frame, max_points, C.byref(prm), float(elev_thresh),
                                             1 if include_dyn else 0, pend_T, pend_ends, n_pend, self._ws_elev.data_ptr(),
                                             self._ws_elev.numel(), elev.data_ptr(), obs.data_ptr(), flags.data_ptr(),
                                             counts.data_ptr(), ctx.stream()))
        self._k1_noted = None
        lo_hi = self.frame_off[[self.head + first_frame, self.head + last_frame]].cpu()
        lo, n = int(lo_hi[0]), min(int(lo_hi[1] - lo_hi[0]), max_points)
        flags = flags[:n]
        if mark_dyn:
            self.dyn[lo + torch.nonzero(flags == 1).squeeze(1)] = 1
        return {'elev': elev, 'observed': obs.bool(), 'flags': flags, 'counts': counts}

    def bev_many(self, jobs, out16):
        ctx, lib = self.ctx, self.ctx.lib
        n = len(jobs)
        if n == 0:
            return out16
        self.flush_pending()
        px = int(jobs[0][1].px)
        assert out16.dtype == torch.float16 and out16.is_contiguous() and tuple(out16.shape) == (n, 21, px, px)
        max_points = self.max_window_points()
        per = (int(lib.pca_bev_workspace_bytes(max_points, px)) + 255) & ~255
        need = per * n + 512
        if self._ws_many is None or self._ws_many.numel() < need:
            self._ws_many = torch.empty(int(need * 1.25), dtype=torch.uint8, device=self.device)
        cj = (_lib.PcaBevJob * n)()
        plane_bytes = 21 * px * px * 2
        for k, (split, prm, first, last) in enumerate(jobs):
            last = self.n_frames if last is None else last
            cj[k].slot_begin, cj[k].slot_split, cj[k].slot_end = self.head + first, self.head + split, self.head + last
            C.memmove(C.addressof(cj[k].prm), C.addressof(prm), C.sizeof(PcaBevParams))
            cj[k].planes = None
            cj[k].planes_f16 = out16.data_ptr() + k * plane_bytes
        st = self.c_store()
        ctx.check(lib.pca_bev_generate_many(ctx.h, C.byref(st), None, self.frame_off.data_ptr(), cj, n, max_points,
                                            self._ws_many.data_ptr(), self._ws_many.numel(), ctx.stream()))
        return out16

    def rows(self, frame=None):
        self.flush_pending()
        off = self.offsets()
        lo, hi = (int(off[0]), int(off[-1])) if frame is None else (int(off[frame]), int(off[frame + 1]))
        out = np.empty((hi - lo, 10))
        out[:, 0] = self.x[lo:hi].cpu().numpy()
        out[:, 1] = self.y[lo:hi].cpu().numpy()
        out[:, 2] = self.z[lo:hi].cpu().numpy()
        i = self.intensity[lo:hi].cpu().numpy().astype(np.float64)
        out[:, 3] = i / 255. if self.intensity_div255 else i
        r = self.rgbs[lo:hi].cpu().numpy().view(np.uint32)
        out[:, 4], out[:, 5], out[:, 6], out[:, 7] = r & 255, (r >> 8) & 255, (r >> 16) & 255, r >> 24
        out[:, 8] = self.inst[lo:hi].cpu().numpy()
        out[:, 9] = self.dyn[lo:hi].cpu().numpy()
        return out

    def frame_rows(self):
        off = self.offsets()
        allrows = self.rows()
        base = int(off[0])
        return [allrows[int(off[k]) - base:int(off[k + 1]) - base] for k in range(self.n_frames)]

    def load_rows(self, rows_list, intensity64_out=None):
        self.clear()
        total = int(sum(r.shape[0] for r in rows_list))
        if total > self.capacity or len(rows_list) > self.max_frames:
            self.max_frames = max(self.max_frames, len(rows_list))
            self._alloc(max(total, 1))
            self.frame_off = torch.zeros(self.max_frames + 1, dtype=torch.int64, device=self.device)
            self._alloc_frame_tables(self.max_frames)
        rows = np.concatenate([np.asarray(r, dtype=np.float64).reshape(-1, 10) for r in rows_list]) if rows_list \
            else np.zeros((0, 10))
        c = rows[:, 4:8]
        if rows.size and not (np.all(c == np.floor(c)) and c.min() >= 0 and c.max() <= 255):
            raise NotImplementedError('rgb / semantic columns must hold integers 0..255')
        if rows.size and not np.all(rows[:, 8] == np.floor(rows[:, 8])):
            raise NotImplementedError('instance column must hold integers')
        d = self.device
        self.x[:total] = torch.from_numpy(np.ascontiguousarray(rows[:, 0])).to(d)
        self.y[:total] = torch.from_numpy(np.ascontiguousarray(rows[:, 1])).to(d)
        self.z[:total] = torch.from_numpy(np.ascontiguousarray(rows[:, 2])).to(d)
        inten = rows[:, 3]
        raw = np.rint(inten * 255.) if self.intensity_div255 else inten
        raw32 = raw.astype(np.float32)
        back = raw32.astype(np.float64) / 255. if self.intensity_div255 else raw32.astype(np.float64)
        i64 = None
        if not np.array_equal(back, inten) or (inten.size and (inten.min() < 0 or np.signbit(inten).any())):
            i64 = torch.from_numpy(np.ascontiguousarray(inten)).to(d)
        self.intensity[:total] = torch.from_numpy(raw32).to(d)
        cu = c.astype(np.uint32)
        packed = (cu[:, 0] | (cu[:, 1] << 8) | (cu[:, 2] << 16) | (cu[:, 3] << 24)).astype(np.uint32)
        self.rgbs[:total] = torch.from_numpy(packed.view(np.int32)).to(d)
        self.inst[:total] = torch.from_numpy(rows[:, 8].astype(np.int32)).to(d)
        self.dyn[:total] = torch.from_numpy((rows[:, 9] == 1).astype(np.uint8)).to(d)
        off = np.concatenate([[0], np.cumsum([r.shape[0] for r in rows_list])]).astype(np.int64)
        self.frame_off[:off.size] = torch.from_numpy(off).to(d)
        self.head, self.tail = 0, len(rows_list)
        self.lb_head, self.ub_tail = 0, total
        self._ub = [int(r.shape[0]) for r in rows_list]
        self._ub_sum = sum(self._ub)
        return i64


def make_bev_params(origin, R, dx, dy, view, px, height_filter, int_scaler, int_sep_scaler, int_mid_threshold,
                    road_class, dynobj_classes, intensity_div255, rgb_fill=0.):
    prm = PcaBevParams()
    prm.origin[:] = [float(v) for v in origin]
    prm.R[:] = [float(v) for v in np.asarray(R, dtype=np.float64).ravel()]
    prm.dx, prm.dy, prm.view = float(dx), float(dy), float(view)
    prm.height_filter = float('nan') if height_filter is None else float(height_filter)
    prm.int_scaler = float(int_scaler)
    prm.int_sep_scaler = float(int_sep_scaler)
    prm.int_mid_threshold = float(int_mid_threshold)
    prm.rgb_fill = float(rgb_fill)
    prm.px = int(px)
    prm.road_class = int(road_class)
    prm.dynobj_mask[:] = list(_lib.class_mask(dynobj_classes))
    prm.intensity_div255 = int(bool(intensity_div255))
    return prm
```

Baseline: 1565 Mpoints/s.

## Move per-frame store bookkeeping into a C session state to cut Python overhead

Adds a C-side pca_store_state that holds the window bookkeeping (head/tail, point counts, pending retransforms, cone and box hints, calibration) plus new pca_store_integrate and pca_store_generate_bev entry points. The Python driver now calls these once per frame instead of doing that bookkeeping in Python. Box readback becomes an async D2H that is polled with an event. The aim is to cut per-frame host and ctypes overhead, at the cost of duplicating state between Python and C, which risks the two copies drifting apart.

```diff
diff --git a/include/pca.h b/include/pca.h
--- a/include/pca.h
+++ b/include/pca.h
@@ -269,6 +269,22 @@
     int32_t hinted, pad2;
 } pca_kitti_generate_bev_args;
 int pca_kitti_generate_bev_v(pca_ctx *ctx, pca_kitti_generate_bev_args *a);
+
+typedef struct pca_store_state pca_store_state;
+typedef struct { int64_t evicted; double path_length; int32_t flags, code, status, pad; } pca_store_integrate_out;
+typedef struct { int32_t n_rows, hinted; } pca_store_generate_bev_out;
+int pca_store_state_bytes(void);
+void pca_store_state_release(pca_store_state *state);
+void pca_store_note_moved(pca_store_state *state, const double T[16]);
+int pca_store_box_poll(pca_ctx *ctx, pca_store_state *state);
+int pca_store_box_start(pca_ctx *ctx, pca_store_state *state, const pca_store *store, void *stream);
+int pca_store_integrate(pca_ctx *ctx, pca_store_state *state, const pca_store *store, int64_t *frame_off ,
+                        const pca_kitti_obs *obs, pca_host_track *track, const double *T_new_prev, double horizon, void *stream,
+                        pca_store_integrate_out *out);
+int pca_store_generate_bev(pca_ctx *ctx, pca_store_state *state, const pca_store *store, int64_t *frame_off , int split,
+                           const pca_bev_params *prm, void *workspace , int64_t workspace_bytes,
+                           uint16_t *planes_f16 , void *host_planes , const pca_host_track *track,
+                           double *traj_rows, int32_t *traj_start, void *stream, pca_store_generate_bev_out *out);
 
 int pca_host_stage_h2d(int n, const void *const *src, void *const *pinned, void *const *dev, const int64_t *bytes,
                        void *stream);
diff --git a/pc-accumulation-lib_amd/csrc/pca_session.hip b/pc-accumulation-lib_amd/csrc/pca_session.hip
--- a/pc-accumulation-lib_amd/csrc/pca_session.hip
+++ b/pc-accumulation-lib_amd/csrc/pca_session.hip
@@ -1,6 +1,7 @@
 #include <vector>
 
 #include "pca_common.h"
+#include "pca_store_state.h"
 
 int pca_stage_copy(const void *const *src, void *const *dst, const int64_t *bytes, int n);
 
@@ -137,4 +138,130 @@
                                   &a->n_rows, a->stream);
 }
 
-}
+
+int pca_store_state_bytes(void) { return (int)sizeof(pca_store_state); }
+
+void pca_store_note_moved(pca_store_state *state, const double *T) { if (state && T) pca_state_note_moved(state, T); }
+
+int pca_store_box_poll(pca_ctx *ctx, pca_store_state *st)
+{
+    if (!ctx || !st) return -1;
+    if (!st->box_in_flight) return 0;
+    const hipError_t e = hipEventQuery((hipEvent_t)st->box_event);
+    if (e == hipErrorNotReady) return 0;
+    PCA_CHECK(ctx, e);
+    pca_state_take_in_boxes(st, (const uint32_t *)st->box_pin);
+    return 1;
+}
+
+int pca_store_box_start(pca_ctx *ctx, pca_store_state *st, const pca_store *store, void *stream)
+{
+    if (!ctx || !st || !store) return -1;
+    if (!pca_state_box_due(st)) return 0;
+    hipStream_t s = (hipStream_t)stream;
+    PCA_CHECK(ctx, hipSetDevice(ctx->device));
+    const int64_t rows = (int64_t)st->max_frames + 1;
+    if (!st->box_pin || st->box_pin_rows < rows) {
+        if (st->box_pin) PCA_CHECK(ctx, hipHostFree(st->box_pin));
+        st->box_pin = nullptr; st->box_pin_rows = 0;
+        PCA_CHECK(ctx, hipHostMalloc(&st->box_pin, (size_t)(24 * rows)));
+        st->box_pin_rows = rows;
+    }
+    if (!st->box_event) {
+        hipEvent_t ev;
+        PCA_CHECK(ctx, hipEventCreateWithFlags(&ev, hipEventDisableTiming));
+        st->box_event = ev;
+    }
+    const int n = st->tail - st->head;
+    PCA_CHECK(ctx, hipMemcpyAsync(st->box_pin, (const char *)store->frame_box + 24ll * st->head, (size_t)(24ll * n),
+                                  hipMemcpyDeviceToHost, s));
+    PCA_CHECK(ctx, hipEventRecord((hipEvent_t)st->box_event, s));
+    pca_state_box_started(st);
+    return 1;
+}
+
+void pca_store_state_release(pca_store_state *st)
+{
+    if (!st) return;
+    if (st->box_event) {
+        if (st->box_in_flight) (void)hipEventSynchronize((hipEvent_t)st->box_event);
+        (void)hipEventDestroy((hipEvent_t)st->box_event);
+    }
+    if (st->box_pin) (void)hipHostFree(st->box_pin);
+    st->box_event = nullptr; st->box_pin = nullptr; st->box_pin_rows = 0; st->box_in_flight = 0;
+}
+
+static int store_flush_owed(pca_ctx *ctx, pca_store_state *st, const pca_store *store, int64_t *frame_off, void *stream)
+{
+    pca_state_flush_plan plan;
+    pca_state_flush_plan_take(st, &plan);
+    for (int r = 0; r < plan.n_ranges; ++r)
+        if (pca_retransform(ctx, store, frame_off, plan.begin[r], plan.end[r], plan.T + 16 * plan.first_T[r],
+                            plan.n_T - plan.first_T[r], stream) != 0)
+            return -1;
+    return 0;
+}
+
+int pca_store_integrate(pca_ctx *ctx, pca_store_state *st, const pca_store *store, int64_t *frame_off, const pca_kitti_obs *obs,
+                        pca_host_track *track, const double *T_new_prev, double horizon, void *stream, pca_store_integrate_out *out)
+{
+    if (!ctx) return -1;
+    if (!st || !store || !frame_off || !obs || obs->n < 0 || !out || !st->k1_set) { ctx->err = "store_integrate: bad arguments"; return -1; }
+    if (!track || !T_new_prev) { ctx->err = "store_integrate: needs the pose track and T_new_prev"; return -1; }
+    out->code = 0; out->evicted = 0; out->status = 0;
+    if (!pca_state_reserve_check(st, obs->n, 1)) { out->code = 1; return 0; }
+    if ((out->flags & 1) && pca_state_n_frames(st) > 0) {
+        if (st->n_pending >= PCA_STATE_CHAIN_MAX && store_flush_owed(ctx, st, store, frame_off, stream)) return -1;
+        pca_state_note_transform(st, T_new_prev);
+    }
+    const int slot = st->tail;
+    if (pca_kitti_integrate(ctx, obs, st->k1_P, st->k1_H, st->k1_W, st->k1_filter, store, frame_off, slot, st->k1_sample_mode, track,
+                            T_new_prev, horizon, &out->evicted, &out->path_length, stream) != 0)
+        return -1;
+    if (pca_state_note_frame(st, slot, obs->sem_gt ? nullptr : st->k1_P, st->k1_H, st->k1_W))
+        pca_host_camera_cone(st->cone_P, st->cone_H, st->cone_W, st->cone);
+    if (pca_store_box_poll(ctx, st) < 0) return -1;
+    if (pca_store_box_start(ctx, st, store, stream) < 0) return -1;
+    pca_state_count_frame(st, obs->n);
+    if (out->evicted) pca_state_evict(st, out->evicted);
+    uint32_t bits = 0;
+    pca_status_peek(ctx, &bits);
+    out->status = (int32_t)bits;
+    return 0;
+}
+
+int pca_store_generate_bev(pca_ctx *ctx, pca_store_state *st, const pca_store *store, int64_t *frame_off, int split,
+                           const pca_bev_params *prm, void *workspace, int64_t workspace_bytes, uint16_t *planes_f16,
+                           void *host_planes, const pca_host_track *track, double *traj_rows, int32_t *traj_start, void *stream,
+                           pca_store_generate_bev_out *out)
+{
+    if (!ctx) return -1;
+    if (!st || !store || !frame_off || !prm || !planes_f16 || !track || !traj_rows || !traj_start || !out) { ctx->err = "store_generate_bev: bad arguments"; return -1; }
+    const int n = pca_state_n_frames(st);
+    out->n_rows = 0; out->hinted = 0;
+    if (pca_host_track_len(track) != n) { ctx->err = "store_generate_bev: the pose track and the window disagree about the number of frames"; return -1; }
+    int n_pend = 0, write_back = 1;
+    if (pca_state_chain_for_raster(st, 0, n, &n_pend, &write_back)) {
+        if (store_flush_owed(ctx, st, store, frame_off, stream)) return -1;
+        n_pend = 0; write_back = 1;
+    }
+    int hinted = 0, slot0 = 0;
+    const double *then = nullptr, *cone = nullptr, *now = nullptr;
+    const float *box = nullptr;
+    const int hint_F = pca_state_hint_args(st, 0, n, &slot0, &then, &box, &cone, &now);
+    if (hint_F > 0 && !(n_pend > 0 && write_back)) {
+        hinted = pca_bev_view_hint(ctx, slot0, hint_F, then, box, cone, now, prm);
+        if (hinted < 0) { ctx->err = "store_generate_bev: bad view hint"; return -1; }
+    }
+    const int ticket = pca_kitti_generate_bev(ctx, store, frame_off, st->head, st->head + split, st->head + n,
+                                              pca_state_max_window_points(st), prm, st->ras_T, st->ras_end, n_pend, write_back,
+                                              workspace, workspace_bytes, planes_f16, host_planes, track, traj_rows, traj_start,
+                                              &out->n_rows, stream);
+    if (ticket < 0) return -1;
+    st->hints_taken += hinted;
+    out->hinted = hinted;
+    pca_state_raster_done(st, write_back);
+    return ticket;
+}
+
+}
diff --git a/pc-accumulation-lib_amd/csrc/pca_store_state.h b/pc-accumulation-lib_amd/csrc/pca_store_state.h
--- /dev/null
+++ b/pc-accumulation-lib_amd/csrc/pca_store_state.h
@@ -0,0 +1,207 @@
+#pragma once
+#include <math.h>
+#include <stdint.h>
+#include <string.h>
+
+#define PCA_STATE_CHAIN_MAX 4
+#define PCA_STATE_BOX_EVERY 16
+
+typedef struct pca_store_state {
+    int32_t head, tail;
+    int32_t max_frames;
+    int32_t chain_k;
+    int64_t capacity;
+    int64_t lb_head, ub_tail;
+    int64_t ub_sum;
+    int64_t *ub;
+    double *then;
+    float *box;
+    uint8_t *has_cone;
+    int32_t n_pending, pad0;
+    double pend_T[16 * PCA_STATE_CHAIN_MAX];
+    int32_t pend_end[PCA_STATE_CHAIN_MAX];
+    double moved[16];
+    int32_t n_nocone;
+    int32_t cone_set;
+    double cone[15];
+    double cone_P[12];
+    int32_t cone_H, cone_W;
+    int32_t since_box;
+    int32_t box_in_flight, box_first, box_n;
+    int32_t cull;
+    int32_t box_every;
+    int64_t hints_taken;
+    int32_t k1_set, k1_H, k1_W, k1_sample_mode;
+    double k1_P[12];
+    uint64_t k1_filter[4];
+    double ras_T[16 * PCA_STATE_CHAIN_MAX];
+    int32_t ras_end[PCA_STATE_CHAIN_MAX];
+    void *box_pin;
+    int64_t box_pin_rows;
+    void *box_event;
+} pca_store_state;
+
+typedef struct pca_state_flush_plan {
+    int32_t n_ranges, n_T;
+    int32_t begin[PCA_STATE_CHAIN_MAX], end[PCA_STATE_CHAIN_MAX], first_T[PCA_STATE_CHAIN_MAX];
+    double T[16 * PCA_STATE_CHAIN_MAX];
+} pca_state_flush_plan;
+
+static inline int pca_state_n_frames(const pca_store_state *s) { return s->tail - s->head; }
+static inline int64_t pca_state_max_window_points(const pca_store_state *s) { return s->ub_sum > 1 ? s->ub_sum : 1; }
+
+static inline int pca_state_reserve_check(const pca_store_state *s, int64_t n_new, int n_slots)
+{
+    return (int64_t)s->tail + n_slots <= s->max_frames && s->ub_tail + n_new <= s->capacity;
+}
+
+static inline void pca_state_note_moved(pca_store_state *s, const double *T)
+{
+    double M[16];
+    for (int r = 0; r < 3; ++r)
+        for (int c = 0; c < 4; ++c) {
+            double acc = T[4 * r] * s->moved[c];
+            for (int k = 1; k < 4; ++k) acc = acc + T[4 * r + k] * s->moved[4 * k + c];
+            M[4 * r + c] = acc;
+        }
+    M[12] = 0.; M[13] = 0.; M[14] = 0.; M[15] = 1.;
+    memcpy(s->moved, M, sizeof M);
+}
+
+static inline int pca_state_note_transform(pca_store_state *s, const double *T)
+{
+    if (s->tail == s->head) return 0;
+    if (s->n_pending >= PCA_STATE_CHAIN_MAX) return -1;
+    pca_state_note_moved(s, T);
+    memcpy(s->pend_T + 16 * s->n_pending, T, 16 * sizeof(double));
+    s->pend_end[s->n_pending++] = s->tail;
+    return 1;
+}
+
+static inline void pca_state_flush_plan_take(pca_store_state *s, pca_state_flush_plan *p)
+{
+    p->n_ranges = 0;
+    p->n_T = s->n_pending;
+    memcpy(p->T, s->pend_T, sizeof p->T);
+    int begin = s->head;
+    for (int k = 0; k < s->n_pending; ++k)
+        if (s->pend_end[k] > begin) {
+            p->begin[p->n_ranges] = begin; p->end[p->n_ranges] = s->pend_end[k]; p->first_T[p->n_ranges] = k;
+            ++p->n_ranges;
+            begin = s->pend_end[k];
+        }
+    s->n_pending = 0;
+}
+
+static inline int pca_state_note_frame(pca_store_state *s, int slot, const double *P, int H, int W)
+{
+    int new_camera = 0;
+    memcpy(s->then + 12 * (size_t)slot, s->moved, 12 * sizeof(double));
+    if (P) {
+        if (!s->cone_set || memcmp(s->cone_P, P, sizeof s->cone_P) != 0 || s->cone_H != H || s->cone_W != W) {
+            if (s->cone_set) {
+                for (int k = s->head; k < s->tail; ++k) s->has_cone[k] = 0;
+                s->n_nocone = s->tail - s->head;
+            }
+            memcpy(s->cone_P, P, sizeof s->cone_P);
+            s->cone_H = H; s->cone_W = W;
+            s->cone_set = 1;
+            new_camera = 1;
+        }
+        s->has_cone[slot] = 1;
+    } else {
+        s->n_nocone += 1;
+    }
+    s->since_box += 1;
+    return new_camera;
+}
+
+static inline int pca_state_box_due(const pca_store_state *s)
+{
+    return s->since_box >= s->box_every && !s->box_in_flight && s->tail > s->head;
+}
+
+static inline void pca_state_box_started(pca_store_state *s)
+{
+    s->box_in_flight = 1; s->box_first = s->head; s->box_n = s->tail - s->head;
+    s->since_box = 0;
+}
+
+static inline float pca_state_f32_from_ordered(uint32_t o)
+{
+    const uint32_t u = o ^ ((o >> 31) ? 0x80000000u : 0xffffffffu);
+    float f;
+    memcpy(&f, &u, sizeof f);
+    return f;
+}
+
+static inline void pca_state_take_in_boxes(pca_store_state *s, const uint32_t *rows)
+{
+    if (!s->box_in_flight) return;
+    s->box_in_flight = 0;
+    for (int f = 0; f < s->box_n; ++f) {
+        float dec[6];
+        for (int k = 0; k < 3; ++k) {
+            const uint32_t l = rows[6 * f + 2 * k], h = rows[6 * f + 2 * k + 1];
+            dec[2 * k] = h != 0u ? pca_state_f32_from_ordered(~l) : 1.0f;
+            dec[2 * k + 1] = h != 0u ? pca_state_f32_from_ordered(h) : -1.0f;
+        }
+        if (dec[0] <= dec[1]) memcpy(s->box + 6 * (size_t)(s->box_first + f), dec, sizeof dec);
+    }
+}
+
+static inline void pca_state_count_frame(pca_store_state *s, int64_t n)
+{
+    s->ub[s->tail] = n;
+    s->tail += 1;
+    s->ub_tail += n;
+    s->ub_sum += n;
+}
+
+static inline void pca_state_evict(pca_store_state *s, int64_t k)
+{
+    if (k > s->tail - s->head) k = s->tail - s->head;
+    if (k <= 0) return;
+    if (s->n_nocone) {
+        int c = 0;
+        for (int64_t j = s->head; j < s->head + k; ++j) c += !s->has_cone[j] && isfinite(s->then[12 * (size_t)j]);
+        s->n_nocone -= c;
+    }
+    for (int64_t j = s->head; j < s->head + k; ++j) s->ub_sum -= s->ub[j];
+    s->head += (int32_t)k;
+}
+
+static inline int pca_state_chain_for_raster(pca_store_state *s, int first_frame, int last_frame, int *n_pend, int *write_back)
+{
+    *n_pend = 0; *write_back = 1;
+    if (s->n_pending == 0) return 0;
+    if (first_frame != 0 || s->pend_end[s->n_pending - 1] > s->head + last_frame) return 1;
+    int n = 0;
+    for (int k = 0; k < s->n_pending; ++k)
+        if (s->pend_end[k] > s->head) {
+            memcpy(s->ras_T + 16 * n, s->pend_T + 16 * k, 16 * sizeof(double));
+            s->ras_end[n++] = s->pend_end[k];
+        }
+    *n_pend = n;
+    *write_back = n == 0 ? 0 : (n >= s->chain_k ? 1 : 0);
+    return 0;
+}
+
+static inline void pca_state_raster_done(pca_store_state *s, int write_back)
+{
+    if (s->n_pending && write_back) s->n_pending = 0;
+}
+
+static inline int pca_state_hint_args(const pca_store_state *s, int first_frame, int last_frame, int *slot0, const double **then,
+                                      const float **box, const double **cone, const double **now)
+{
+    const int n = last_frame - first_frame;
+    if (!s->cull || n < 4) return 0;
+    const int a = s->head + first_frame;
+    *slot0 = a;
+    *then = s->then + 12 * (size_t)a;
+    *box = s->box + 6 * (size_t)a;
+    *cone = (s->cone_set && s->n_nocone == 0) ? s->cone : nullptr;
+    *now = s->moved;
+    return n;
+}
diff --git a/pc-accumulation-lib_amd/kitti360_sem_pc_accum.py b/pc-accumulation-lib_amd/kitti360_sem_pc_accum.py
--- a/pc-accumulation-lib_amd/kitti360_sem_pc_accum.py
+++ b/pc-accumulation-lib_amd/kitti360_sem_pc_accum.py
@@ -36,6 +36,7 @@
         self._ga_traj = None
         self._fast = os.environ.get('PCA_FAST_CALLS', '1') != '0'
         self._defer_k1 = self._fast and os.environ.get('PCA_FUSE_K1', '1') != '0'
+        self._session = self._fast and os.environ.get('PCA_KITTI_SESSION', '1') != '0'
         self._prev_sweep = None
         self._sweep_dev = None
         self.pose_provider = self._default_pose_provider()
@@ -193,6 +194,8 @@
         rgb, pc, sem_gt = observations[0]
         if not self.use_gt_sem:
             sem_gt = None
+        if self._session and self._store is not None and self._store._k1_noted is not None:
+            self._store.flush_k1()
         T_new_prev = np.asarray(self.pose_provider(pc), dtype=np.float64)
         self.T_prev_origin = np.matmul(self.T_prev_origin, T_new_prev)
         if self._sweep_dev is not None:
@@ -202,6 +205,25 @@
                 pc = dev
         fast = self._obs_pointers(rgb, pc, sem_gt) if self._fast else None
         general = self._frame_tensors(rgb, pc, sem_gt) if fast is None else None
+        if fast is not None and self._session and getattr(self._track, '_h', None) is not None:
+            obs, semseg, H, W, keep = fast
+            store = self.store
+            if self._defer_k1 != getattr(store.ctx, 'k1_defer', False):
+                store.set_defer_k1(self._defer_k1)
+            idx, path_length = store.integrate_obs(obs, self.P_velo_frame, H, W, self.semseg_filters, self.sample_mode, self._track,
+                                                   T_new_prev, self.horizon_dist, len(self._track) > 0, keep=keep)
+            del keep
+            self.rgbs.append(rgb)
+            self.semsegs.append(semseg)
+            if idx:
+                self.rgbs = self.rgbs[idx:]
+                self.semsegs = self.semsegs[idx:]
+            if path_length is not None:
+                print(f'    #pc {store.n_frames} |', f'path length {path_length:.2f}')
+            self._integrated += 1
+            if self.voxel_dedup and self._integrated % max(self.voxel_dedup_every, 1) == 0:
+                store.voxel_dedup(self.voxel_dedup)
+            return idx
         if len(self._track) > 0:
             self.update_sem_pcs(T_new_prev)
         if fast is not None:
@@ -328,6 +350,19 @@
         rot_mat = hl.rotation_matrix_3d(hl.heading_rot_ang(near[:split - lo] - origin))
         px = gen.pixel_size
         prm = gen._raster_params(origin, rot_mat, 0., 0., 1. * gen.view_size, st.intensity_div255)
+        if self._session:
+            if out is None:
+                out = torch.empty((21, px, px), dtype=torch.float16, device=st.device)
+            else:
+                assert out.dtype == torch.float16 and out.is_contiguous() and tuple(out.shape) == (21, px, px)
+            host = torch.empty((1, 21, px, px), dtype=torch.float16, pin_memory=True) if to_host else None
+            tb = self._ga_traj
+            if tb is None or tb[0].shape[0] < 2 * n or tb[1].shape[0] < n + 1:
+                tb = self._ga_traj = (np.empty((4 * n + 64, 3)), np.zeros(2 * n + 64, dtype=np.int32))
+                self._ga_traj_addr = (tb[0].ctypes.data, tb[1].ctypes.data)
+            ticket, n_rows = st.raster_kitti(split, prm, out.data_ptr(), None if host is None else host.data_ptr(), track,
+                                             *self._ga_traj_addr)
+            return self._bev_result(tb, n_rows, split, n, out, host, ticket, to_host)
         max_points = st.bev_workspace(px)
         n_pend, pend_T, pend_ends, write_back = st.bev_pending(0, n)
         if out is None:
@@ -366,7 +401,12 @@
             ctx.check(ticket)
         st.hints_taken += a.hinted
         st.bev_done(write_back)
-        rows = tb[0][:a.n_rows].copy()
+        return self._bev_result(tb, a.n_rows, split, n, out, host, ticket, to_host)
+
+    def _bev_result(self, tb, n_rows, split, n, out, host, ticket, to_host):
+        _, _, LazyBev, _PendingCopy, _, _, _ = _mods()
+        ctx, start = self.store.ctx, tb[1]
+        rows = tb[0][:n_rows].copy()
         empty = np.zeros((0, 3))
         ego_p = rows[:start[split - 1]].copy() if split >= 2 else empty
         ego_f = rows[start[split]:].copy() if n - split >= 2 else empty
diff --git a/pc-accumulation-lib_amd/pca_amd/_lib.py b/pc-accumulation-lib_amd/pca_amd/_lib.py
--- a/pc-accumulation-lib_amd/pca_amd/_lib.py
+++ b/pc-accumulation-lib_amd/pca_amd/_lib.py
@@ -25,7 +25,7 @@
            'pca_host_track_append', 'pca_host_track_push_segment', 'pca_host_track_incr', 'pca_host_track_evict_beyond',
            'pca_host_track_step', 'pca_host_track_trigger', 'pca_host_stage_h2d', 'pca_host_d2h_async', 'pca_host_d2h_wait',
            'pca_deflate_workspace_bytes', 'pca_deflate_chunks', 'pca_host_crc32_combine', 'pca_host_gzip_assemble',
-           'pca_kitti_integrate', 'pca_kitti_generate_bev', 'pca_k1_defer', 'pca_k1_flush', 'pca_host_camera_cone', 'pca_host_view_hull', 'pca_bev_bin_range', 'pca_bev_view_hint', 'pca_kitti_integrate_v', 'pca_kitti_generate_bev_v', 'pca_f32_box_decode', 'pca_debug_bev_level1', 'pca_debug_icp_layout',
+           'pca_kitti_integrate', 'pca_kitti_generate_bev', 'pca_k1_defer', 'pca_k1_flush', 'pca_host_camera_cone', 'pca_host_view_hull', 'pca_bev_bin_range', 'pca_bev_view_hint', 'pca_kitti_integrate_v', 'pca_kitti_generate_bev_v', 'pca_f32_box_decode', 'pca_store_state_bytes', 'pca_store_state_release', 'pca_store_note_moved', 'pca_store_box_poll', 'pca_store_box_start', 'pca_store_integrate', 'pca_store_generate_bev', 'pca_debug_bev_level1', 'pca_debug_icp_layout',
            'pca_profile_enable', 'pca_profile_read')
 
 KERNEL_IDS = ('kitti_project_sample_filter', 'nusc_sample_filter_transform', 'nusc_project_cams', 'retransform',
@@ -55,6 +55,32 @@
                 ('pad1', C.c_int32), ('stream', C.c_void_p), ('hint_slot0', C.c_int32), ('hint_F', C.c_int32),
                 ('hint_then', C.c_void_p), ('hint_box', C.c_void_p), ('hint_cone', C.c_void_p), ('hint_now', C.c_void_p),
                 ('hinted', C.c_int32), ('pad2', C.c_int32)]
+
+
+class PcaStoreState(C.Structure):
+    CHAIN_MAX = 4
+    _fields_ = [('head', C.c_int32), ('tail', C.c_int32), ('max_frames', C.c_int32), ('chain_k', C.c_int32),
+                ('capacity', C.c_int64), ('lb_head', C.c_int64), ('ub_tail', C.c_int64), ('ub_sum', C.c_int64),
+                ('ub', C.c_void_p), ('then', C.c_void_p), ('box', C.c_void_p), ('has_cone', C.c_void_p),
+                ('n_pending', C.c_int32), ('pad0', C.c_int32), ('pend_T', C.c_double * (16 * CHAIN_MAX)),
+                ('pend_end', C.c_int32 * CHAIN_MAX), ('moved', C.c_double * 16),
+                ('n_nocone', C.c_int32), ('cone_set', C.c_int32), ('cone', C.c_double * 15), ('cone_P', C.c_double * 12),
+                ('cone_H', C.c_int32), ('cone_W', C.c_int32), ('since_box', C.c_int32), ('box_in_flight', C.c_int32),
+                ('box_first', C.c_int32), ('box_n', C.c_int32), ('cull', C.c_int32), ('box_every', C.c_int32),
+                ('hints_taken', C.c_int64),
+                ('k1_set', C.c_int32), ('k1_H', C.c_int32), ('k1_W', C.c_int32), ('k1_sample_mode', C.c_int32),
+                ('k1_P', C.c_double * 12), ('k1_filter', C.c_uint64 * 4),
+                ('ras_T', C.c_double * (16 * CHAIN_MAX)), ('ras_end', C.c_int32 * CHAIN_MAX),
+                ('box_pin', C.c_void_p), ('box_pin_rows', C.c_int64), ('box_event', C.c_void_p)]
+
+
+class PcaStoreIntegrateOut(C.Structure):
+    _fields_ = [('evicted', C.c_int64), ('path_length', C.c_double), ('flags', C.c_int32), ('code', C.c_int32),
+                ('status', C.c_int32), ('pad', C.c_int32)]
+
+
+class PcaStoreGenerateBevOut(C.Structure):
+    _fields_ = [('n_rows', C.c_int32), ('hinted', C.c_int32)]
 
 
 class PcaKittiObs(C.Structure):
@@ -243,6 +269,16 @@
     lib.pca_bev_view_hint.argtypes = [vp, i32, i32, vp, vp, vp, vp, vp]
     lib.pca_f32_box_decode.argtypes = [vp, i32, vp]
     lib.pca_f32_box_decode.restype = None
+    lib.pca_store_state_release.argtypes = [vp]
+    lib.pca_store_state_release.restype = None
+    lib.pca_store_note_moved.argtypes = [vp, vp]
+    lib.pca_store_note_moved.restype = None
+    lib.pca_store_box_poll.argtypes = [vp, vp]
+    lib.pca_store_box_start.argtypes = [vp, vp, vp, vp]
+    lib.pca_store_integrate.argtypes = [vp, vp, vp, vp, vp, vp, vp, C.c_double, vp, vp]
+    lib.pca_store_generate_bev.argtypes = [vp, vp, vp, vp, i32, vp, vp, i64, vp, vp, vp, vp, vp, vp, vp]
+    if lib.pca_store_state_bytes() != C.sizeof(PcaStoreState):
+        raise RuntimeError('libpca_hip.so and pca_amd._lib disagree about pca_store_state: rebuild the library')
     lib.pca_debug_bev_level1.argtypes = [vp, vp]
     lib.pca_debug_icp_layout.argtypes = [i32, i32, C.POINTER(C.c_int64)]
     lib.pca_kitti_integrate_v.argtypes = [vp, vp]
diff --git a/pc-accumulation-lib_amd/pca_amd/device_store.py b/pc-accumulation-lib_amd/pca_amd/device_store.py
--- a/pc-accumulation-lib_amd/pca_amd/device_store.py
+++ b/pc-accumulation-lib_amd/pca_amd/device_store.py
@@ -1,37 +1,147 @@
 import ctypes as C
 import os
+import sys
 
 import numpy as np
 import torch
 
 from . import _lib
-from ._lib import PcaBevParams, PcaKittiFrame, PcaStore
+from ._lib import PcaBevParams, PcaKittiFrame, PcaStore, PcaStoreState
 
 CULL = os.environ.get('PCA_BEV_CULL', '1') != '0'
+
+
+def _state_int(name):
+    return property(lambda self: getattr(self._sb, name), lambda self, v: setattr(self._sb, name, int(v)))
+
+
+class _OwedChain:
+    __slots__ = ('_sb', )
+
+    def __init__(self, sb):
+        self._sb = sb
+
+    def __len__(self):
+        return self._sb.n_pending
+
+    def _index(self, k):
+        n = self._sb.n_pending
+        k = k + n if k < 0 else k
+        if not 0 <= k < n:
+            raise IndexError('owed chain index out of range')
+        return k
+
+    def __getitem__(self, k):
+        k = self._index(k)
+        return np.array(self._sb.pend_T[16 * k:16 * k + 16]), int(self._sb.pend_end[k])
+
+    def __setitem__(self, k, item):
+        k = self._index(k)
+        T, end = item
+        self._sb.pend_T[16 * k:16 * k + 16] = [float(v) for v in np.asarray(T, dtype=np.float64).reshape(16)]
+        self._sb.pend_end[k] = int(end)
+
+    def __iter__(self):
+        return iter([self[k] for k in range(len(self))])
+
+    def __eq__(self, other):
+        mine = [self[k] for k in range(len(self))]
+        return len(mine) == len(other) and all(np.array_equal(a[0], b[0]) and a[1] == b[1] for a, b in zip(mine, other))
+
+    def append(self, item):
+        if self._sb.n_pending >= PcaStoreState.CHAIN_MAX:
+            raise IndexError('the owed chain is full')
+        self._sb.n_pending += 1
+        self[self._sb.n_pending - 1] = item
+
+    def __repr__(self):
+        return repr([self[k] for k in range(len(self))])
 
 
 class DeviceStore:
     CHAIN_MAX = 4
-    CHAIN_K = int(os.environ.get('PCA_BEV_CHAIN', '4'))
+    CHAIN_K_DEFAULT = int(os.environ.get('PCA_BEV_CHAIN', '4'))
+
+    head = _state_int('head')
+    tail = _state_int('tail')
+    ub_tail = _state_int('ub_tail')
+    lb_head = _state_int('lb_head')
+    capacity = _state_int('capacity')
+    max_frames = _state_int('max_frames')
+    hints_taken = _state_int('hints_taken')
+    _ub_sum = _state_int('ub_sum')
+    _n_nocone = _state_int('n_nocone')
+    _since_box = _state_int('since_box')
+    CHAIN_K = _state_int('chain_k')
+    cull = property(lambda self: bool(self._sb.cull), lambda self, v: setattr(self._sb, 'cull', int(bool(v))))
+
+    @property
+    def _moved(self):
+        return self._moved_np
+
+    @_moved.setter
+    def _moved(self, M):
+        self._moved_np[...] = np.asarray(M, dtype=np.float64).reshape(4, 4)
+
+    @property
+    def _ub(self):
+        return self._ub_np[self.head:self.tail].tolist()
+
+    @_ub.setter
+    def _ub(self, sizes):
+        self._ub_np[self.head:self.head + len(sizes)] = np.asarray(sizes, dtype=np.int64)
+
+    @property
+    def _pending(self):
+        return _OwedChain(self._sb)
+
+    @_pending.setter
+    def _pending(self, items):
+        items = list(items)
+        assert len(items) <= self.CHAIN_MAX
+        self._sb.n_pending = len(items)
+        chain = _OwedChain(self._sb)
+        for k, item in enumerate(items):
+            chain[k] = item
+
+    @property
+    def _cone(self):
+        sb = self._sb
+        if not sb.cone_set:
+            return None
+        return (bytes(sb.cone_P), sb.cone_H, sb.cone_W), self._cone_np, self._cone_addr
+
+    @_cone.setter
+    def _cone(self, cone):
+        if cone is None:
+            self._sb.cone_set = 0
+            return
+        key, sb = cone[0], self._sb
+        C.memmove(C.addressof(sb.cone_P), key[0], 96)
+        sb.cone_H, sb.cone_W = int(key[1]), int(key[2])
+        self.ctx.lib.pca_host_camera_cone(C.addressof(sb.cone_P), sb.cone_H, sb.cone_W, self._cone_addr)
+        sb.cone_set = 1
 
     def __init__(self, capacity=1 << 24, max_frames=4096, device=None, intensity_div255=False):
         self.ctx = _lib.Context.get(device)
         self.device = torch.device('cuda', self.ctx.device_index)
         self.intensity_div255 = bool(intensity_div255)
+        sb = self._sb = PcaStoreState()
+        self._sb_addr = C.addressof(sb)
+        self._owed_T_addr, self._ras_T_addr = self._sb_addr + PcaStoreState.pend_T.offset, self._sb_addr + PcaStoreState.ras_T.offset
+        sb.chain_k, sb.box_every = self.CHAIN_K_DEFAULT, self.BOX_EVERY
+        self._moved_np = np.frombuffer(sb, dtype=np.float64, count=16, offset=PcaStoreState.moved.offset).reshape(4, 4)
+        self._moved_addr = self._moved_np.ctypes.data
+        self._cone_np = np.frombuffer(sb, dtype=np.float64, count=15, offset=PcaStoreState.cone.offset)
+        self._cone_addr = self._cone_np.ctypes.data
         self.max_frames = int(max_frames)
         self._alloc(int(capacity))
         self.frame_off = torch.zeros(self.max_frames + 1, dtype=torch.int64, device=self.device)
         self._moved = np.eye(4)
         self.cull = CULL
-        self.hints_taken = 0
         self._alloc_frame_tables(self.max_frames)
-        self.head = 0
-        self.tail = 0
-        self.ub_tail = 0
-        self.lb_head = 0
-        self._ub = []
-        self._ub_sum = 0
-        self._pending = []
+        self._io = None
+        self._go = None
         self._k1_cache = None
         self._k1_src = None
         self._ia = None
@@ -45,9 +155,8 @@
         self._dedup_ws = None
         self._obs_out = None
         self._k1_noted = None
-        self._pend_T = (C.c_double * (16 * self.CHAIN_MAX))()
-        self._pend_T_np = np.frombuffer(self._pend_T, dtype=np.float64)
-        self._pend_ends = (C.c_int * self.CHAIN_MAX)()
+        self._pend_T = sb.ras_T
+        self._pend_ends = sb.ras_end
 
     def _alloc(self, cap):
         d = self.device
@@ -72,63 +181,49 @@
         then = np.full((n1, 12), np.nan)
         seen = np.tile(np.array([1, -1] * 3, dtype=np.float32), (n1, 1))
         cone = np.zeros(n1, dtype=bool)
+        ub = np.zeros(n1, dtype=np.int64)
         if keep is not None:
             a, n = keep
             box[:n] = self.frame_box[a:a + n]
-            then[:n], seen[:n], cone[:n] = self._then[a:a + n], self._box[a:a + n], self._has_cone[a:a + n]
-        self.frame_box, self._then, self._box, self._has_cone = box, then, seen, cone
+            then[:n], seen[:n], cone[:n], ub[:n] = self._then[a:a + n], self._box[a:a + n], self._has_cone[a:a + n], self._ub_np[a:a + n]
+        else:
+            self._cone = None
+        self.frame_box, self._then, self._box, self._has_cone, self._ub_np = box, then, seen, cone, ub
         self._then_addr, self._box_addr = then.ctypes.data, seen.ctypes.data
-        self._box_pin = None
-        self._box_copy = None
+        sb = self._sb
+        sb.then, sb.box, sb.has_cone, sb.ub = self._then_addr, self._box_addr, cone.ctypes.data, ub.ctypes.data
+        sb.box_in_flight = 0
         self._since_box = 0
-        self._cone = None
         self._n_nocone = 0 if keep is None else int(np.count_nonzero(~cone[:keep[1]] & np.isfinite(then[:keep[1], 0])))
         self._cstore = None
 
     def _note_moved(self, Ts):
-        for T in Ts:
-            M = T.reshape(4, 4) @ self._moved
-            M[3] = (0., 0., 0., 1.)
-            self._moved = M
+        note, base = self.ctx.lib.pca_store_note_moved, Ts.ctypes.data
+        for k in range(Ts.shape[0]):
+            note(self._sb_addr, base + 128 * k)
 
     def _note_frame(self, slot, cone_key):
         self._then[slot] = self._moved[:3].reshape(12)
         if cone_key is not None:
-            if self._cone is None or self._cone[0] != cone_key:
-                if self._cone is not None:
+            cone = self._cone
+            if cone is None or cone[0] != cone_key:
+                if cone is not None:
                     self._has_cone[self.head:self.tail] = False
                     self._n_nocone = self.tail - self.head
-                out = np.empty(15)
-                Pm = np.frombuffer(cone_key[0], dtype=np.float64)
-                self.ctx.lib.pca_host_camera_cone(Pm.ctypes.data, int(cone_key[1]), int(cone_key[2]), out.ctypes.data)
-                self._cone = (cone_key, out, out.ctypes.data)
+                self._cone = (cone_key, )
             self._has_cone[slot] = True
         else:
             self._n_nocone += 1
         self._since_box += 1
+        self._sb.box_every = self.BOX_EVERY
         self._poll_boxes()
-        if self._since_box >= self.BOX_EVERY and self._box_copy is None:
-            n = self.tail - self.head
-            if n > 0:
-                if self._box_pin is None or self._box_pin.shape[0] < self.frame_box.shape[0]:
-                    self._box_pin = torch.empty(tuple(self.frame_box.shape), dtype=torch.int32, pin_memory=True)
-                self._box_pin[:n].copy_(self.frame_box[self.head:self.tail], non_blocking=True)
-                ev = torch.cuda.Event()
-                ev.record()
-                self._box_copy = (ev, self.head, n)
-                self._since_box = 0
+        st, ctx = self.c_store(), self.ctx
+        if ctx.lib.pca_store_box_start(ctx.h, self._sb_addr, C.addressof(st), ctx.stream_int() or None) < 0:
+            ctx.check(-1)
 
     def _poll_boxes(self):
-        if self._box_copy is None or not self._box_copy[0].query():
-            return
-        _, first, n = self._box_copy
-        self._box_copy = None
-        rows = self._box_pin[:n].numpy()
-        dec = np.empty((n, 6), dtype=np.float32)
-        self.ctx.lib.pca_f32_box_decode(rows.ctypes.data, n, dec.ctypes.data)
-        known = dec[:, 0] <= dec[:, 1]
-        tgt = self._box[first:first + n]
-        tgt[known] = dec[known]
+        if self._sb.box_in_flight and self.ctx.lib.pca_store_box_poll(self.ctx.h, self._sb_addr) < 0:
+            self.ctx.check(-1)
 
     def view_hint_into(self, args, first_frame, last_frame):
         n = last_frame - first_frame
@@ -138,7 +233,7 @@
         args.hint_slot0 = a
         args.hint_then, args.hint_box = self._then_addr + 96 * a, self._box_addr + 24 * a
         args.hint_cone = self._cone[2] if (self._cone is not None and self._n_nocone == 0) else None
-        args.hint_now = self._moved.ctypes.data
+        args.hint_now = self._moved_addr
         return n
 
     def view_hint(self, prm, first_frame, last_frame, write_back):
@@ -148,7 +243,7 @@
         a = self.head + first_frame
         cone = self._cone[2] if (self._cone is not None and self._n_nocone == 0) else None
         return self._count_hint(self.ctx.lib.pca_bev_view_hint(self.ctx.h, a, n, self._then_addr + 96 * a, self._box_addr + 24 * a, cone,
-                                              self._moved.ctypes.data, C.addressof(prm)))
+                                              self._moved_addr, C.addressof(prm)))
 
     def _count_hint(self, r):
         self.hints_taken += 1 if r > 0 else 0
@@ -182,14 +277,19 @@
                 self.flush_k1()
         except Exception:
             pass
+        try:
+            if not sys.is_finalizing():
+                self.ctx.lib.pca_store_state_release(self._sb_addr)
+        except Exception:
+            pass
 
     def offsets(self):
         self.flush_k1()
         off = self.frame_off[self.head:self.tail + 1].cpu().numpy()
         self.lb_head = int(off[0])
         self.ub_tail = int(off[-1])
-        self._ub = [int(v) for v in np.diff(off)]
-        self._ub_sum = sum(self._ub)
+        self._ub_np[self.head:self.tail] = np.diff(off)
+        self._ub_sum = int(off[-1]) - int(off[0])
         return off
 
     def sizes(self):
@@ -226,9 +326,7 @@
         new_off = torch.zeros(new_maxf + 1, dtype=torch.int64, device=self.device)
         new_off[:nf + 1] = torch.from_numpy(off - a).to(self.device)
         self.frame_off = new_off
-        cone = self._cone
         self._alloc_frame_tables(new_maxf, keep=(self.head, nf))
-        self._cone = cone
         self.head, self.tail = 0, nf
         self.lb_head, self.ub_tail = 0, live
 
@@ -237,9 +335,8 @@
         if self._n_nocone and k:
             sl = slice(self.head, self.head + k)
             self._n_nocone -= int(np.count_nonzero(~self._has_cone[sl] & np.isfinite(self._then[sl, 0])))
+        self._ub_sum -= int(self._ub_np[self.head:min(self.head + k, self.tail)].sum())
         self.head += k
-        self._ub_sum -= sum(self._ub[:int(k)])
-        del self._ub[:int(k)]
 
     def max_window_points(self):
         return max(self._ub_sum, 1)
@@ -248,7 +345,6 @@
         self.flush_k1()
         self.head = self.tail = 0
         self.ub_tail = self.lb_head = 0
-        self._ub = []
         self._ub_sum = 0
         self._pending = []
         self.frame_off.zero_()
@@ -275,22 +371,17 @@
         if descs is None:
             descs = self.kitti_descs(frames)
         st = self.c_store()
-        key = (np.asarray(P, dtype=np.float64).tobytes(), tuple(int(c) for c in (filters or ())))
-        if self._k1_cache is None or self._k1_cache[0] != key:
-            self._k1_cache = (key, _lib.f64_array(P, 12), _lib.class_mask(filters))
+        self._k1_calibration(P, filters)
         Pc, fmask = self._k1_cache[1], self._k1_cache[2]
         ctx.check(lib.pca_kitti_project_sample_filter_ex(ctx.h, descs, len(frames), Pc, int(H), int(W),
                                                          fmask, C.byref(st), self.frame_off.data_ptr(), self.tail,
                                                          _lib.SAMPLE_MODES[sample_mode], ctx.stream()))
+        self._ub_np[self.tail:self.tail + len(frames)] = [int(f['pts'].shape[0]) for f in frames]
         self.tail += len(frames)
         self.ub_tail += n_in
-        self._ub += [int(f['pts'].shape[0]) for f in frames]
         self._ub_sum += n_in
 
-    def append_kitti_obs(self, obs, P, H, W, filters, sample_mode='nearest', track=None, T_new_prev=None, horizon=0., keep=None):
-        lib, ctx = self.ctx.lib, self.ctx
-        n = int(obs.n)
-        self.reserve(n, 1)
+    def _k1_calibration(self, P, filters):
         src = self._k1_src
         if src is not None and src[0] is P and src[1] is filters and P.tobytes() == src[2] and tuple(filters or ()) == src[3]:
             key = self._k1_cache[0]
@@ -300,7 +391,77 @@
             self._k1_src = (P, filters, key[0], key[1]) if ok else None
         if self._k1_cache is None or self._k1_cache[0] != key:
             self._k1_cache = (key, _lib.f64_array(P, 12), _lib.class_mask(filters))
+            sb = self._sb
+            C.memmove(C.addressof(sb.k1_P), self._k1_cache[1], 96)
+            C.memmove(C.addressof(sb.k1_filter), self._k1_cache[2], 32)
+            sb.k1_set = 1
+        return key
+
+    def integrate_obs(self, obs, P, H, W, filters, sample_mode, track, T_new_prev, horizon, owe_T, keep=None):
+        lib, ctx, sb = self.ctx.lib, self.ctx, self._sb
+        self._k1_calibration(P, filters)
+        sb.k1_H, sb.k1_W, sb.k1_sample_mode, sb.box_every = int(H), int(W), _lib.SAMPLE_MODES[sample_mode], self.BOX_EVERY
+        io = self._io
+        if io is None:
+            io = self._io = [_lib.PcaStoreIntegrateOut(), np.zeros(16), None, None]
+        o, T = io[0], io[1]
+        T[:] = np.asarray(T_new_prev, dtype=np.float64).reshape(16)
+        th = track._h
+        for attempt in (0, 1):
+            st = self.c_store()
+            const = (id(obs), id(st), id(self.frame_off), th)
+            if const != io[2]:
+                io[2] = const
+                io[3] = (C.addressof(st), self.frame_off.data_ptr(), C.addressof(obs), getattr(th, 'value', th), T.ctypes.data,
+                         C.addressof(o), (obs, st, self.frame_off))
+            a = io[3]
+            o.flags = 1 if owe_T else 0
+            if lib.pca_store_integrate(ctx.h, self._sb_addr, a[0], a[1], a[2], a[3], a[4], float(horizon), ctx.stream_int() or None, a[5]):
+                ctx.check(-1)
+            if o.code == 0:
+                break
+            if attempt:
+                raise RuntimeError('pca: the store has no room for the frame after making room for it')
+            if owe_T:
+                self.retransform(T.reshape(4, 4), defer=True)
+                owe_T = False
+            self.reserve(int(obs.n), 1)
+        self._k1_noted = (keep, ) if getattr(ctx, 'k1_defer', False) else None
+        if o.status:
+            ctx.check_status()
+        v = o.path_length
+        return int(o.evicted), (None if v != v else np.float64(v))
+
+    def raster_kitti(self, split, prm, planes_ptr, host_ptr, track, traj_rows_addr, traj_start_addr):
+        lib, ctx, sb = self.ctx.lib, self.ctx, self._sb
+        px = int(prm.px)
+        if self._ws is None or max(sb.ub_sum, 1) > self._ws_points or px != self._ws_px:
+            self.bev_workspace(px)
+        go = self._go
+        if go is None:
+            go = self._go = [_lib.PcaStoreGenerateBevOut(), None, None]
+        o = go[0]
+        st, th = self.c_store(), track._h
+        const = (id(st), id(self.frame_off), id(self._ws), th)
+        if const != go[1]:
+            go[1] = const
+            go[2] = (C.addressof(st), self.frame_off.data_ptr(), self._ws.data_ptr(), self._ws.numel(), getattr(th, 'value', th),
+                     C.addressof(o), (st, self.frame_off, self._ws))
+        a = go[2]
+        ticket = lib.pca_store_generate_bev(ctx.h, self._sb_addr, a[0], a[1], int(split), C.addressof(prm), a[2], a[3], planes_ptr,
+                                            host_ptr, a[4], traj_rows_addr, traj_start_addr, ctx.stream_int() or None, a[5])
+        if ticket < 0:
+            ctx.check(ticket)
+        self._k1_noted = None
+        return ticket, o.n_rows
+
+    def append_kitti_obs(self, obs, P, H, W, filters, sample_mode='nearest', track=None, T_new_prev=None, horizon=0., keep=None):
+        lib, ctx = self.ctx.lib, self.ctx
+        n = int(obs.n)
+        self.reserve(n, 1)
+        key = self._k1_calibration(P, filters)
         Pc, fmask = self._k1_cache[1], self._k1_cache[2]
+        self._sb.k1_H, self._sb.k1_W, self._sb.k1_sample_mode = int(H), int(W), _lib.SAMPLE_MODES[sample_mode]
         st = self.c_store()
         th = getattr(track, '_h', None)
         a = self._ia
@@ -326,9 +487,9 @@
         ctx.check(lib.pca_kitti_integrate_v(ctx.h, C.addressof(a)))
         self._k1_noted = (keep, ) if getattr(ctx, 'k1_defer', False) else None
         self._note_frame(self.tail, (key[0], int(H), int(W)) if obs.sem_gt is None else None)
+        self._ub_np[self.tail] = n
         self.tail += 1
         self.ub_tail += n
-        self._ub.append(n)
         self._ub_sum += n
         if th is None:
             return None, None
@@ -346,9 +507,9 @@
                                                           _lib.f64_array(T, 16), _lib.class_mask(filters),
                                                           C.byref(st), self.frame_off.data_ptr(), self.tail,
                                                           _lib.SAMPLE_MODES[sample_mode], ctx.stream()))
+        self._ub_np[self.tail] = n
         self.tail += 1
         self.ub_tail += n
-        self._ub.append(n)
         self._ub_sum += n
 
     def append_nusc_many(self, frames, filters, sample_mode='nearest'):
@@ -386,9 +547,9 @@
             ctx.check(lib.pca_nusc_sample_filter_transform_batch(ctx.h, descs, len(part), ncam, H, W, _lib.class_mask(filters),
                                                                  C.byref(st), self.frame_off.data_ptr(), self.tail,
                                                                  _lib.SAMPLE_MODES[sample_mode], ctx.stream()))
+            self._ub_np[self.tail:self.tail + len(part)] = [int(f['pc'].shape[0]) for f in part]
             self.tail += len(part)
             self.ub_tail += n_in
-            self._ub += [int(f['pc'].shape[0]) for f in part]
             self._ub_sum += n_in
             b0 = b1
 
@@ -398,9 +559,13 @@
         Ts = np.ascontiguousarray(Ts, dtype=np.float64).reshape(-1, 16)
         self._note_moved(Ts)
         if defer and Ts.shape[0] == 1:
-            if len(self._pending) >= self.CHAIN_MAX:
+            sb = self._sb
+            if sb.n_pending >= self.CHAIN_MAX:
                 self.flush_pending()
-            self._pending.append((Ts[0].copy(), self.tail))
+            k = sb.n_pending
+            C.memmove(self._owed_T_addr + 128 * k, Ts.ctypes.data, 128)
+            sb.pend_end[k] = self.tail
+            sb.n_pending = k + 1
             return
         self.flush_pending()
         self._launch_retransform(Ts, self.head, self.tail)
@@ -426,7 +591,8 @@
                                                      _lib.f64_array(Ts, Ts.size), ctx.stream()))
 
     def flush_pending(self):
-        pend, self._pending = self._pending, []
+        pend = list(self._pending)
+        self._sb.n_pending = 0
         begin = self.head
         for k, (_, end_slot) in enumerate(pend):
             if end_slot > begin:
@@ -493,24 +659,25 @@
         return max_points
 
     def bev_pending(self, first_frame, last_frame):
-        if not self._pending:
+        sb = self._sb
+        if not sb.n_pending:
             return 0, None, None, 1
-        if first_frame != 0 or self._pending[-1][1] > self.head + last_frame:
+        if first_frame != 0 or sb.pend_end[sb.n_pending - 1] > self.head + last_frame:
             self.flush_pending()
             return 0, None, None, 1
-        n_pend = 0
-        for T, e in self._pending:
-            if e > self.head:
-                self._pend_T_np[16 * n_pend:16 * n_pend + 16] = T
-                self._pend_ends[n_pend] = int(e)
+        n_pend, head, ends = 0, self.head, sb.pend_end
+        for k in range(sb.n_pending):
+            if ends[k] > head:
+                C.memmove(self._ras_T_addr + 128 * n_pend, self._owed_T_addr + 128 * k, 128)
+                self._pend_ends[n_pend] = ends[k]
                 n_pend += 1
         if n_pend == 0:
             return 0, None, None, 0
         return n_pend, self._pend_T, self._pend_ends, (1 if n_pend >= self.CHAIN_K else 0)
 
     def bev_done(self, write_back):
-        if self._pending and write_back:
-            self._pending = []
+        if self._sb.n_pending and write_back:
+            self._sb.n_pending = 0
         self._k1_noted = None
 
     def bev_class_planes(self, split_frame, prm, groups, first_frame=0, last_frame=None, want_counts=False):
@@ -659,7 +826,7 @@
         self.head, self.tail = 0, len(rows_list)
         self.lb_head, self.ub_tail = 0, total
         self._ub = [int(r.shape[0]) for r in rows_list]
-        self._ub_sum = sum(self._ub)
+        self._ub_sum = total
         return i64
 
 
```

After: 1573 Mpoints/s (median of 2 runs). Within noise of the previous version (+0.5%).
